# zhen6618/EPRecon

Measured on AMD Instinct MI355X. Metric: fragments_per_sec, higher is better.
Workload: dtype f32

## Files before the change

### eprecon_amd/_lib.py

```python
import ctypes
import os

import numpy as np
import torch

_HERE = os.path.dirname(os.path.abspath(__file__))
LIB_PATH = os.environ.get("EPRECON_LIB_PATH") or os.path.join(_HERE, "libeprecon_hip.so")

_c = ctypes
_vp, _i, _i64, _f, _sz = _c.c_void_p, _c.c_int, _c.c_int64, _c.c_float, _c.c_size_t

SIGNATURES = {
    "eprecon_abi_version": (_i, []),
    "eprecon_build_arch": (_c.c_char_p, []),
    "eprecon_back_project_workspace_bytes": (_sz, [_i64, _i, _i, _i, _i, _i, _i]),
    "eprecon_back_project_async": (_i, [_vp, _i64, _vp, _i, _f, _vp, _i, _vp, _i, _i, _i, _i, _i, _i,
                                        _vp, _vp, _vp, _vp, _vp, _vp, _vp, _vp, _sz, _vp]),
    "eprecon_back_project_call_async": (_i, [_vp, _vp]),
    "eprecon_back_project_call": (_i, [_vp, _i, _vp, _vp]),
    "eprecon_back_project_prepare_levels_async": (_i, [_vp, _i, _vp]),
    "eprecon_back_project_workspace_maps_offset": (_sz, [_i64, _i]),
    "eprecon_bp_levels": (_i, []),
    "eprecon_init_glue": (_i, []),
    "eprecon_profile_gather_kernel": (_c.c_char_p, []),
    "eprecon_hash_capacity": (_c.c_uint32, [_i64]),
    "eprecon_hash_table_bytes": (_sz, [_c.c_uint32]),
    "eprecon_hash_build_async": (_i, [_vp, _i64, _i, _vp, _c.c_uint32, _vp]),
    "eprecon_hash_build_dn_async": (_i, [_vp, _i64, _vp, _i, _vp, _c.c_uint32, _vp]),
    "eprecon_hash_query_async": (_i, [_vp, _c.c_uint32, _vp, _i64, _i, _vp, _vp]),
    "eprecon_hash_status": (_i, [_vp, _vp]),
    "eprecon_unique_workspace_bytes": (_sz, [_i64]),
    "eprecon_unique_coords_async": (_i, [_vp, _i64, _i, _vp, _c.c_uint32, _vp, _vp, _vp, _vp, _sz, _vp]),
    "eprecon_unique_coords_dn_async": (_i, [_vp, _i64, _vp, _i, _vp, _c.c_uint32, _vp, _vp, _vp, _vp, _sz, _vp]),
    "eprecon_unique_hierarchy_dn_async": (_i, [_vp, _i64, _vp, _i, _vp, _vp, _vp, _vp, _vp, _vp, _sz, _vp]),
    "eprecon_point_quantize_dn_async": (_i, [_vp, _i64, _vp, _f, _vp, _vp, _vp]),
    "eprecon_spvcnn_points_dn_async": (_i, [_vp, _i64, _vp, _i, _i, _vp, _i, _f, _vp, _f, _vp, _vp, _vp, _vp, _vp, _vp]),
    "eprecon_gru_stage_capacity": (_i64, [_vp, _i64, _i]),
    "eprecon_gru_stage_workspace_bytes": (_sz, [_i64]),
    "eprecon_gru_stage_begin_async": (_i, [_vp, _vp]),
    "eprecon_gru_stage_commit_async": (_i, [_vp, _vp, _vp, _vp]),
    "eprecon_kernel_map_async": (_i, [_vp, _c.c_uint32, _vp, _i64, _i, _i, _vp, _vp]),
    "eprecon_kernel_map_self_async": (_i, [_vp, _c.c_uint32, _vp, _i64, _i, _vp, _vp]),
    "eprecon_components_workspace_bytes": (_sz, [_i64]),
    "eprecon_components_async": (_i, [_vp, _i64, _vp, _i, _vp, _vp, _vp, _sz, _vp]),
    "eprecon_transpose_map_async": (_i, [_vp, _i64, _vp, _i, _vp, _vp]),
    "eprecon_sparse_conv_async": (_i, [_vp, _i64, _i, _vp, _i, _i64, _vp, _i, _i, _vp, _vp, _i, _i, _i, _vp]),
    "eprecon_conv_bn_partial_bytes": (_sz, [_i64, _i]),
    "eprecon_sparse_conv_fused_async": (_i, [_vp, _i64, _i, _vp, _i, _i64, _vp, _i, _i, _vp, _vp, _i, _vp, _i, _i, _i,
                                             _vp, _vp]),
    "eprecon_conv_desc_async": (_i, [_vp, _vp]),
    "eprecon_exclusive_scan_scratch_ints": (_sz, [_i64]),
    "eprecon_exclusive_scan_async": (_i, [_vp, _i64, _vp, _vp, _vp, _vp]),
    "eprecon_conv_desc_partial_rows": (_i64, [_vp]),
    "eprecon_conv_dense3d_kind": (_i, [_vp]),
    "eprecon_bn_acc_words": (_sz, [_i]),
    "eprecon_conv_desc_takes_bn_acc": (_i, [_vp]),
    "eprecon_batchnorm_acc_affine_async": (_i, [_vp, _i, _i, _i, _f, _vp, _vp, _vp]),
    "eprecon_affine_rows_acc_async": (_i, [_vp, _i64, _i, _i, _vp, _i, _i, _f, _i, _vp, _i, _vp]),
    "eprecon_affine_rows_res_async": (_i, [_vp, _i64, _i, _i, _vp, _vp, _vp, _i, _i, _vp, _i, _vp]),
    "eprecon_batchnorm_finalize_affine_async": (_i, [_vp, _i64, _i64, _i, _vp, _vp, _f, _vp, _vp, _vp]),
    "eprecon_affine_rows_async": (_i, [_vp, _i64, _i, _i, _vp, _vp, _i, _vp, _i, _vp]),
    "eprecon_affine_pool2_rows_async": (_i, [_vp, _i, _i, _i, _i, _i, _vp, _vp, _i, _vp, _i, _vp]),
    "eprecon_affine_up2_rows_async": (_i, [_vp, _i, _i, _i, _i, _i, _vp, _vp, _i, _vp, _i, _vp]),
    "eprecon_pixel_map_async": (_i, [_i, _i, _i, _i, _vp, _vp]),
    "eprecon_batchnorm_apply_workspace_bytes": (_sz, [_i]),
    "eprecon_batchnorm_apply_partials_async": (_i, [_vp, _i64, _i, _i, _vp, _i64, _i64, _vp, _vp, _f, _vp, _i, _i, _vp, _i,
                                                    _vp, _vp, _vp, _sz, _vp]),
    "eprecon_batchnorm_apply_partials_res_async": (_i, [_vp, _i64, _i, _i, _vp, _i64, _i64, _vp, _vp, _f, _vp, _i, _vp, _vp, _i,
                                                        _vp, _i, _vp, _sz, _vp]),
    "eprecon_batchnorm_workspace_bytes": (_sz, [_i64, _i]),
    "eprecon_batchnorm_train_async": (_i, [_vp, _i64, _i, _i, _vp, _vp, _f, _vp, _i, _i, _vp, _i, _vp, _vp,
                                           _vp, _sz, _vp]),
    "eprecon_rowwise_layernorm_async": (_i, [_vp, _i64, _i, _i, _vp, _i, _vp, _vp, _f, _i, _i, _vp, _i, _vp]),
    "eprecon_init_select_workspace_bytes": (_sz, [_i, _i]),
    "eprecon_init_select_async": (_i, [_vp, _vp, _i64, _f, _i, _i, _i, _vp, _vp, _vp, _sz, _vp]),
    "eprecon_init_select_dense_async": (_i, [_vp, _vp, _i64, _vp, _i, _i, _i, _i, _f, _i, _i, _vp, _vp, _vp, _sz, _vp]),
    "eprecon_upsample_async": (_i, [_vp, _i, _vp, _i64, _i, _i, _vp, _vp, _vp]),
    "eprecon_aligned_coords_async": (_i, [_vp, _i64, _vp, _i, _f, _vp, _vp, _vp]),
    "eprecon_point_quantize_async": (_i, [_vp, _i64, _f, _vp, _vp, _vp]),
    "eprecon_segment_workspace_bytes": (_sz, [_i64, _i64]),
    "eprecon_segment_lists_async": (_i, [_vp, _i64, _i64, _vp, _vp, _vp, _sz, _vp]),
    "eprecon_segment_mean_async": (_i, [_vp, _i, _vp, _vp, _i64, _i, _vp, _i, _vp]),
    "eprecon_sphash_async": (_i, [_vp, _i64, _vp, _vp]),
    "eprecon_sphash_order_workspace_bytes": (_sz, [_i64]),
    "eprecon_sphash_order_async": (_i, [_vp, _i64, _vp, _vp, _vp, _sz, _vp]),
    "eprecon_remap_index_async": (_i, [_vp, _i64, _vp, _vp, _i64, _vp, _vp]),
    "eprecon_trilinear_map_async": (_i, [_vp, _c.c_uint32, _vp, _i64, _i, _vp, _vp, _vp]),
    "eprecon_devoxelize_async": (_i, [_vp, _i, _vp, _vp, _i64, _i, _vp, _i, _i, _vp]),
    "eprecon_sparse_conv_wgrad_workspace_bytes": (_sz, [_i, _i64, _i, _i]),
    "eprecon_sparse_conv_wgrad_async": (_i, [_vp, _i, _vp, _i, _vp, _i, _i64, _i, _i, _vp, _vp, _sz, _vp]),
    "eprecon_invert_map_async": (_i, [_vp, _i, _i64, _i64, _vp, _vp]),
    "eprecon_devoxelize_backward_async": (_i, [_vp, _i, _vp, _vp, _i64, _i, _i64, _vp, _i, _vp]),
    "eprecon_gather_rows_scaled_async": (_i, [_vp, _i, _vp, _vp, _i64, _i, _vp, _i, _vp]),
    "eprecon_back_project_backward_async": (_i, [_vp, _i64, _vp, _i, _f, _vp, _vp, _i, _i, _i, _i, _i, _vp, _i, _vp, _vp, _vp]),
    "eprecon_back_project_backward_workspace_bytes": (_sz, [_i, _i, _i, _i, _i]),
    "eprecon_back_project_backward_det_async": (_i, [_vp, _i64, _vp, _i, _f, _vp, _vp, _i, _i, _i, _i, _i, _vp, _i, _vp, _vp, _vp, _sz,
                                                     _vp]),
    "eprecon_devoxelize_backward_csr_async": (_i, [_vp, _i, _vp, _vp, _vp, _i64, _i, _vp, _i, _vp]),
    "eprecon_devoxelize_gate_async": (_i, [_vp, _i, _vp, _vp, _i64, _i, _vp, _i, _i, _vp, _i, _vp, _i, _vp, _i, _vp]),
    "eprecon_devoxelize_gate_tail_async": (_i, [_vp, _i, _vp, _vp, _i64, _i, _vp, _i, _i, _vp, _i, _vp, _i, _vp, _i, _vp, _i, _vp, _i,
                                                _i, _vp]),
    "eprecon_fbv_union_workspace_bytes": (_sz, [_i]),
    "eprecon_fbv_union_async": (_i, [_vp, _vp, _i64, _i, _vp, _vp, _i64, _i, _i, _i, _i, _i, _vp, _vp, _vp, _vp, _vp,
                                     _vp, _vp, _sz, _vp]),
    "eprecon_map_set_fragment": (_i, [_vp, _i]),
    "eprecon_map_stamps_async": (_i, [_vp, _vp, _vp, _i, _c.c_int32, _vp]),
    "eprecon_map_select_boundary_async": (_i, [_vp, _vp, _i, _i, _i, _vp, _vp]),
    "eprecon_map_pack_boundary_async": (_i, [_vp, _vp, _i64, _vp]),
    "eprecon_map_merge_boundary": (_i, [_vp, _vp, _i64, _vp, _i, _vp, _vp]),
    "eprecon_map_create": (_i, [_i, _c.POINTER(_vp)]),
    "eprecon_map_destroy": (_i, [_vp]),
    "eprecon_map_reset": (_i, [_vp]),
    "eprecon_map_size": (_i64, [_vp]),
    "eprecon_map_channels": (_i, [_vp]),
    "eprecon_map_export_async": (_i, [_vp, _vp, _vp, _vp]),
    "eprecon_map_import_async": (_i, [_vp, _vp, _vp, _i64, _vp]),
    "eprecon_map_crop_union": (_i, [_vp, _vp, _vp, _i64, _i, _i, _i, _i, _vp, _vp, _vp, _vp, _vp, _vp]),
    "eprecon_map_gather_async": (_i, [_vp, _vp, _i64, _i, _i, _f, _vp, _i, _vp]),
    "eprecon_map_update_async": (_i, [_vp, _vp, _i64, _vp, _i, _vp]),
    "eprecon_map_target_fuse": (_i, [_vp, _vp, _vp, _i, _vp, _vp, _i64, _vp, _vp]),
    "eprecon_gather_rows_async": (_i, [_vp, _i, _vp, _i64, _i, _f, _vp, _i, _vp]),
    "eprecon_tsdf_integrate_async": (_i, [_vp, _vp, _vp, _vp, _f, _vp, _i, _i, _i, _vp, _vp, _f, _f, _i, _vp, _vp]),
    "eprecon_gt_crop_async": (_i, [_vp, _vp]),
    "eprecon_label_volumes_workspace_bytes": (_sz, [_i64, _i64]),
    "eprecon_label_volumes": (_i, [_vp, _vp, _vp, _vp, _i64, _vp, _c.c_double, _vp, _vp, _vp, _vp, _vp, _sz, _vp]),
    "eprecon_label_fill_workspace_bytes": (_sz, [_i, _i, _i]),
    "eprecon_label_fill_async": (_i, [_vp, _vp, _vp, _vp, _sz, _vp]),
    "eprecon_marching_cubes_table": (_i, [_vp]),
    "eprecon_marching_cubes_workspace_bytes": (_sz, [_i, _i, _i]),
    "eprecon_marching_cubes_count": (_i, [_vp, _i, _i, _i, _f, _vp, _vp, _sz, _vp]),
    "eprecon_marching_cubes_emit_async": (_i, [_vp, _i, _i, _i, _f, _vp, _vp, _vp, _vp, _vp, _vp, _vp, _vp, _vp]),
    "eprecon_marching_cubes_count_masked": (_i, [_vp, _vp, _i, _i, _i, _f, _vp, _vp, _sz, _vp]),
    "eprecon_marching_cubes_emit_masked_async": (_i, [_vp, _vp, _i, _i, _i, _f, _vp, _vp, _vp, _vp, _vp, _vp, _vp, _vp, _vp]),
# ... 404 lines not shown
```

### eprecon_amd/csrc/conv_common.hpp

```cpp
#pragma once
#include "common.hpp"

namespace epconv {

struct ConvParams {
    const float *x;
    const int32_t *nbr;
    const float *w;
    const float *bias;
    float *out;
    int n_out, K, Cin, Cout, ld_x, ld_out;
    int64_t x_bytes;
    int relu;
    int accumulate;
    const float *res;
    int ld_res;
    float *bn_partial;
    int bn_ld;
    const float *in_scale, *in_shift;
    int in_relu;
    const float *res_scale, *res_shift;
    int res_relu;
    int ln;
    const float *ln_gamma, *ln_beta;
    float ln_eps;
    int ln_post_relu;
    int img_h, img_w, img_maps;
    int flex_partial;
    const int32_t *vox_rank;
    int gx, gy, gz;
    const float *wq;
    const float *wq16;
    int debug;
    int splitk_pipe;
    void *ws;
    size_t ws_bytes;
    long long *bn_acc;
    int bn_acc_ld, bn_acc_c0;
    const float *bn_gamma, *bn_beta;
    const long long *in_acc;
    int in_acc_ld, in_acc_c0;
    float in_eps;
};

constexpr int kBnCopies = 8, kBnWords = 7;
#ifndef EP_BN_ABL
#define EP_BN_ABL 0
#endif

__device__ __forceinline__ void bn_limbs(double x, long long &l0, long long &l1, long long &l2)
{
    const double v = x * 1099511627776.0;
    const double hi = floor(v * (1.0 / 1099511627776.0));
    l0 = (long long)(v - hi * 1099511627776.0);
    const long long h = (long long)hi;
    l1 = h & ((1ll << 40) - 1);
    l2 = h >> 40;
}

__device__ __forceinline__ void bn_acc_add(long long *acc, int ld, int c, int copy, float n, float mean, float m2)
{
    if (n <= 0.0f || (EP_BN_ABL & 1)) return;
    unsigned long long *a = reinterpret_cast<unsigned long long *>(acc) + ((size_t)copy * ld + c) * kBnWords;
    const double dn = (double)n, dm = (double)mean;
    long long l0, l1, l2;
    bn_limbs(dn * dm, l0, l1, l2);
    atomicAdd(a + 0, (unsigned long long)l0);
    if (EP_BN_ABL & 4) return;
    atomicAdd(a + 1, (unsigned long long)l1); atomicAdd(a + 2, (unsigned long long)l2);
    bn_limbs((double)m2 + dn * dm * dm, l0, l1, l2);
    atomicAdd(a + 3, (unsigned long long)l0); atomicAdd(a + 4, (unsigned long long)l1); atomicAdd(a + 5, (unsigned long long)l2);
    atomicAdd(a + 6, (unsigned long long)(long long)n);
}

__device__ __forceinline__ void bn_acc_affine(const long long *acc, int ld, int c, float eps, float &scale, float &shift)
{
    if (EP_BN_ABL & 2) { scale = 1.0f; shift = 0.0f; return; }
    long long w[kBnWords] = {0, 0, 0, 0, 0, 0, 0};
#pragma unroll 1
    for (int k = 0; k < kBnCopies; ++k) {
        const long long *a = acc + ((size_t)k * ld + c) * kBnWords;
#pragma unroll
        for (int j = 0; j < kBnWords; ++j) w[j] += a[j];
    }
    const double two40 = 1099511627776.0;
    const double s1 = ((double)w[2] * two40 + (double)w[1]) + (double)w[0] * (1.0 / two40);
    const double s2 = ((double)w[5] * two40 + (double)w[4]) + (double)w[3] * (1.0 / two40);
    const double n = (double)w[6];
    const float *gb = reinterpret_cast<const float *>(acc + (size_t)kBnCopies * ld * kBnWords);
    const double mean = n > 0.0 ? s1 / n : 0.0;
    double var = n > 0.0 ? s2 / n - mean * mean : 0.0;
    if (var < 0.0) var = 0.0;
    const float sc = gb[c] / sqrtf((float)var + eps);
    scale = sc;
    shift = gb[ld + c] - (float)mean * sc;
}

template <int THREADS, bool ACC = true>
__device__ __forceinline__ void stage_in_affine(const ConvParams &p, float *sAff, int cpad, int tid)
{
    if (!p.in_scale) return;
    for (int c = tid; c < cpad; c += THREADS) {
        float sc = 0.0f, sh = 0.0f;
        if (c < p.Cin) {
            if (ACC && p.in_acc) bn_acc_affine(p.in_acc, p.in_acc_ld, p.in_acc_c0 + c, p.in_eps, sc, sh);
            else { sc = p.in_scale[c]; sh = p.in_shift[c]; }
        }
        sAff[c] = sc;
        sAff[cpad + c] = sh;
    }
}

__device__ __forceinline__ void bn_acc_publish(const ConvParams &p, int col, int copy, bool first, float n, float mean, float m2)
{
    bn_acc_add(p.bn_acc, p.bn_acc_ld, p.bn_acc_c0 + col, copy & (kBnCopies - 1), n, mean, m2);
    if (first) {
        float *gb = reinterpret_cast<float *>(p.bn_acc + (size_t)kBnCopies * p.bn_acc_ld * kBnWords);
        gb[p.bn_acc_c0 + col] = p.bn_gamma ? p.bn_gamma[col] : 1.0f;
        gb[p.bn_acc_ld + p.bn_acc_c0 + col] = p.bn_beta ? p.bn_beta[col] : 0.0f;
    }
}

constexpr int kWaves = 4;
constexpr int kRowsPerWave = 32;
constexpr int kRowsPerBlock = kRowsPerWave * kWaves;
typedef float f32x4 __attribute__((ext_vector_type(4)));
typedef unsigned int u32x4 __attribute__((ext_vector_type(4)));
// ... 72 lines not shown
            }
#pragma unroll
            for (int m = 8; m > 0; m >>= 1) sq += __shfl_xor(sq, m);
            const float inv = 1.0f / sqrtf(sq * inv_c + p.ln_eps);
#pragma unroll
            for (int t = 0; t < CT; ++t) {
                const int col = 16 * t + l16;
                float y = fmaf(v[t][j] * inv, (p.ln_gamma && colok[t]) ? p.ln_gamma[col] : 1.0f, (p.ln_beta && colok[t]) ? p.ln_beta[col] : 0.0f);
                if (p.ln_post_relu) y = fmaxf(y, 0.0f);
                v[t][j] = y;
            }
        }
    }
#pragma unroll
    for (int t = 0; t < CT; ++t)
#pragma unroll
        for (int j = 0; j < 4; ++j)
            if (colok[t] && orow[j] >= 0) p.out[(size_t)orow[j] * p.ld_out + 16 * t + l16] = v[t][j];
    if (p.bn_partial || (ACC && p.bn_acc)) {
#pragma unroll
        for (int t = 0; t < CT; ++t) {
            float n = 0.0f, sum = 0.0f;
#pragma unroll
            for (int j = 0; j < 4; ++j)
                if (orow[j] >= 0) { n += 1.0f; sum += v[t][j]; }
            float mean = n > 0.0f ? sum / n : 0.0f, m2 = 0.0f;
#pragma unroll
            for (int j = 0; j < 4; ++j)
                if (orow[j] >= 0) { const float d = v[t][j] - mean; m2 = fmaf(d, d, m2); }
#pragma unroll
            for (int m = 16; m < 64; m <<= 1) {
                const float on = __shfl_xor(n, m), om = __shfl_xor(mean, m), oq = __shfl_xor(m2, m);
                const bool lower = (lane & m) == 0;
                float a_n = lower ? n : on, a_mean = lower ? mean : om, a_m2 = lower ? m2 : oq;
                chan_merge(a_n, a_mean, a_m2, lower ? on : n, lower ? om : mean, lower ? oq : m2);
                n = a_n; mean = a_mean; m2 = a_m2;
            }
            if (q == 0) {
                float *d = sStat + (wave * 3) * 16 * CT + 16 * t + l16;
                d[0] = n; d[16 * CT] = mean; d[2 * 16 * CT] = m2;
            }
        }
        __syncthreads();
        if (tid < 16 * CT && tid < p.Cout) {
            float a_n = 0.0f, a_mean = 0.0f, a_m2 = 0.0f;
#pragma unroll
            for (int w = 0; w < NW; ++w)
                chan_merge(a_n, a_mean, a_m2, sStat[(w * 3) * 16 * CT + tid], sStat[(w * 3 + 1) * 16 * CT + tid], sStat[(w * 3 + 2) * 16 * CT + tid]);
            if (p.bn_partial) bn_partial_store(p, partial_row, tid, a_n, a_mean, a_m2);
            if (ACC && p.bn_acc) bn_acc_publish(p, tid, partial_row, partial_row == 0, a_n, a_mean, a_m2);
        }
    }
}

inline bool gather_vec4(const ConvParams &p)
{
    return (p.ld_x % 4 == 0) && ((reinterpret_cast<uintptr_t>(p.x) & 15) == 0) && (p.Cin % 4 == 0 || p.ld_x >= ((p.Cin + 3) & ~3));
}

enum D3Kind { kD3None = 0, kD3Narrow = 1, kD3Tile16 = 2 };
__attribute__((visibility("hidden"))) int conv3d_shape_kind(const ConvParams &p);
int conv3d_kind(const ConvParams &p);
int d3_tiles_kind(const ConvParams &p, int kind, int *ty = nullptr, int *tz = nullptr);
int launch_conv3d_16(const ConvParams &p, hipStream_t st);
int launch_conv3d_single_column(const ConvParams &p, hipStream_t st);

bool conv2d_tile_ok(const ConvParams &p, int *nt_out, int *nch_out, int64_t *blocks);
int launch_image_tile(const ConvParams &p, hipStream_t st);

constexpr int kWideRows = 128;
size_t wide_workspace_bytes(const ConvParams &p);
bool wide_shape_ok(const ConvParams &p);
bool wide_ok(const ConvParams &p);
int launch_wide(const ConvParams &p, hipStream_t st);

constexpr int kSplitKRows = 32;
bool splitk_ok(const ConvParams &p);
int launch_splitk(ConvParams &p, hipStream_t st);

bool resident_narrow_ok(const ConvParams &p);
int launch_resident_narrow(const ConvParams &p, hipStream_t st);
bool resident_wide_ok(const ConvParams &p);
int launch_resident_wide(const ConvParams &p, hipStream_t st);
int launch_mfma(const ConvParams &p, hipStream_t st);

bool direct16_ok(const ConvParams &p);
constexpr int kDirectRows = 128;
int launch_direct16(const ConvParams &p, hipStream_t st);
int direct16_partial_block_rows(const ConvParams &p);
size_t direct16_workspace_bytes(const ConvParams &p);

constexpr int kT2MinRows = 40000;
constexpr int kDirectMaxCout = 64;
constexpr int64_t kK1DirectMinRows = 20000;
bool tile2d16_ok(const ConvParams &p);
int64_t tile2d16_partial_rows(const ConvParams &p);
int launch_tile2d16(const ConvParams &p, hipStream_t st);

constexpr int kT2ShortMaxRows = 20000;
bool tile2d_short_list(const ConvParams &p);
bool tile2d_short_ok(const ConvParams &p);
int64_t tile2d_short_partial_rows(const ConvParams &p);
int launch_tile2d_short(const ConvParams &p, hipStream_t st);


}
```

### eprecon_amd/csrc/norm.hip

```cpp
#include <stdlib.h>

#include "common.hpp"
#include "conv_common.hpp"

namespace {
using namespace ep;

constexpr int kBnPerThread = 8;

__device__ __forceinline__ void chan_merge(float &n_a, float &mean_a, float &m2_a, float n_b, float mean_b, float m2_b)
{
    if (n_b == 0.0f) return;
    if (n_a == 0.0f) {
        n_a = n_b; mean_a = mean_b; m2_a = m2_b;
        return;
    }
    const float n = n_a + n_b;
    const float d = mean_b - mean_a;
    mean_a = mean_a + d * (n_b / n);
    m2_a = m2_a + m2_b + d * d * (n_a * n_b / n);
    n_a = n;
}

__global__ __launch_bounds__(256) void bn_stats_kernel(const float *x, int n, int C, int ld, float *partial)
// ... 12 lines not shown
        const bool ok = active && r < n;
        v[k] = ok ? x[(size_t)r * ld + col] : 0.0f;
        cnt += ok ? 1.0f : 0.0f;
        sum += v[k];
    }
    const float mean = cnt > 0.0f ? sum / cnt : 0.0f;
    float m2 = 0.0f;
#pragma unroll
    for (int k = 0; k < kBnPerThread; ++k) {
        const int r = r0 + k * rpi + rsub;
        if (active && r < n) {
            const float d = v[k] - mean;
            m2 = fmaf(d, d, m2);
        }
    }
    sN[tid] = cnt; sMean[tid] = mean; sM2[tid] = m2;
    __syncthreads();
    for (int s = 1; s < rpi; s <<= 1) {
        if (active && (rsub % (2 * s)) == 0 && rsub + s < rpi) {
            float n = sN[tid], m = sMean[tid], q = sM2[tid];
            const int o = tid + s * C;
            chan_merge(n, m, q, sN[o], sMean[o], sM2[o]);
            sN[tid] = n; sMean[tid] = m; sM2[tid] = q;
        }
        __syncthreads();
    }
    if (tid < C) {
        const size_t plane = (size_t)C * gridDim.x;
        float *p = partial + (size_t)tid * gridDim.x + blockIdx.x;
        p[0] = sN[tid]; p[plane] = sMean[tid]; p[2 * plane] = sM2[tid];
    }
}

template <int NU>
__device__ __forceinline__ void bn_merge_rows(const float *partial, int nblk, int64_t ld, int C, int c, int tid, float &a_n,
                                              float &a_mean, float &a_m2)
{
    const float *pn = partial + (size_t)c * ld, *pm = pn + (size_t)C * ld, *pq = pm + (size_t)C * ld;
    for (int b = tid; b < nblk; b += NU * 256) {
        float vn[NU], vm[NU], vq[NU];
#pragma unroll
        for (int u = 0; u < NU; ++u) {
            const int bb = b + u * 256;
            const bool ok = bb < nblk;
            vn[u] = ok ? pn[bb] : 0.0f;
            vm[u] = ok ? pm[bb] : 0.0f;
            vq[u] = ok ? pq[bb] : 0.0f;
        }
#pragma unroll
        for (int u = 0; u < NU; ++u) chan_merge(a_n, a_mean, a_m2, vn[u], vm[u], vq[u]);
    }
}

inline int bn_finalize_nu(int64_t nblk)
{
    const int64_t need = (nblk + 255) / 256;
    return need <= 1 ? 1 : need <= 2 ? 2 : need <= 4 ? 4 : need <= 8 ? 8 : 16;
}

template <int NU>
__global__ __launch_bounds__(256) void bn_finalize_kernel(const float *partial, int nblk, int64_t ld, int C, float *mean_out,
                                                          float *var_out)
{
    __shared__ float sN[256], sMean[256], sM2[256];
    const int c = blockIdx.x, tid = threadIdx.x;
    float a_n = 0.0f, a_mean = 0.0f, a_m2 = 0.0f;
    bn_merge_rows<NU>(partial, nblk, ld, C, c, tid, a_n, a_mean, a_m2);
    sN[tid] = a_n; sMean[tid] = a_mean; sM2[tid] = a_m2;
    __syncthreads();
    for (int s = 128; s > 0; s >>= 1) {
        if (tid < s) {
            float n = sN[tid], m = sMean[tid], q = sM2[tid];
            chan_merge(n, m, q, sN[tid + s], sMean[tid + s], sM2[tid + s]);
            sN[tid] = n; sMean[tid] = m; sM2[tid] = q;
        }
        __syncthreads();
    }
    if (tid == 0) {
        mean_out[c] = sMean[0];
        var_out[c] = sN[0] > 0.0f ? sM2[0] / sN[0] : 0.0f;
    }
}

template <int NU>
__global__ __launch_bounds__(256) void bn_finalize_affine_kernel(const float *partial, int nblk, int64_t ld, int C,
                                                                 const float *gamma, const float *beta, float eps,
                                                                 float *scale_out, float *shift_out)
{
    __shared__ float sN[4], sMean[4], sM2[4];
    const int c = blockIdx.x, tid = threadIdx.x;
    const float g_c = gamma ? gamma[c] : 1.0f, b_c = beta ? beta[c] : 0.0f;
    float a_n = 0.0f, a_mean = 0.0f, a_m2 = 0.0f;
    bn_merge_rows<NU>(partial, nblk, ld, C, c, tid, a_n, a_mean, a_m2);
    const int lane = tid & 63;
#pragma unroll
    for (int m = 1; m < 64; m <<= 1) {
        const float on = __shfl_xor(a_n, m), om = __shfl_xor(a_mean, m), oq = __shfl_xor(a_m2, m);
        float ln = (lane & m) ? on : a_n, lm = (lane & m) ? om : a_mean, lq = (lane & m) ? oq : a_m2;
        chan_merge(ln, lm, lq, (lane & m) ? a_n : on, (lane & m) ? a_mean : om, (lane & m) ? a_m2 : oq);
        a_n = ln; a_mean = lm; a_m2 = lq;
    }
    if (lane == 0) { sN[tid >> 6] = a_n; sMean[tid >> 6] = a_mean; sM2[tid >> 6] = a_m2; }
    __syncthreads();
    if (tid == 0) {
        float n = sN[0], mean = sMean[0], m2 = sM2[0];
        for (int w = 1; w < 4; ++w) chan_merge(n, mean, m2, sN[w], sMean[w], sM2[w]);
        const float var = n > 0.0f ? m2 / n : 0.0f;
        const float sc = g_c / sqrtf(var + eps);
        scale_out[c] = sc;
        shift_out[c] = b_c - mean * sc;
    }
}

__global__ __launch_bounds__(256) void bn_apply_kernel(const float *x, int n, int C, int ld_x,
                                                       const float *mean, const float *var,
                                                       const float *gamma, const float *beta, float eps,
                                                       const float *res, int ld_res, const float *res_scale,
                                                       const float *res_shift, int relu, float *out, int ld_out)
{
    const size_t e = (size_t)blockIdx.x * 256 + threadIdx.x;
    if (e >= (size_t)n * C) return;
    const int r = (int)(e / C), c = (int)(e - (size_t)r * C);
    const float inv = 1.0f / sqrtf(var[c] + eps);
    float v = (x[(size_t)r * ld_x + c] - mean[c]) * inv;
    v = v * (gamma ? gamma[c] : 1.0f) + (beta ? beta[c] : 0.0f);
    if (res) {
        float rv = res[(size_t)r * ld_res + c];
        if (res_scale) rv = fmaf(rv, res_scale[c], res_shift[c]);
        v += rv;
    }
    if (relu) v = fmaxf(v, 0.0f);
    out[(size_t)r * ld_out + c] = v;
}

__global__ __launch_bounds__(256) void rowwise_ln_kernel(const float *x, int n, int C, int ld_x,
                                                         const float *res, int ld_res,
                                                         const float *gamma, const float *beta, float eps,
                                                         int pre_relu, int post_relu, float *out,
                                                         int ld_out)
{
    const int g = threadIdx.x & 7;
    const int r = blockIdx.x * 32 + (threadIdx.x >> 3);
    const bool live = r < n;
    const float *xr = x + (size_t)(live ? r : 0) * ld_x;
    const float *rr = res ? res + (size_t)(live ? r : 0) * ld_res : nullptr;
    auto value = [&](int c) -> float {
        float v = xr[c];
        if (pre_relu) v = fmaxf(v, 0.0f);
        if (rr) v += rr[c];
        return v;
    };
    float s = 0.0f;
    if (live)
        for (int c = g; c < C; c += 8) s += value(c);
    s += __shfl_xor(s, 1);
    s += __shfl_xor(s, 2);
    s += __shfl_xor(s, 4);
    const float mean = s / (float)C;
    float q = 0.0f;
    if (live)
        for (int c = g; c < C; c += 8) {
            const float d = value(c) - mean;
            q = fmaf(d, d, q);
        }
    q += __shfl_xor(q, 1);
    q += __shfl_xor(q, 2);
    q += __shfl_xor(q, 4);
    const float inv = 1.0f / sqrtf(q / (float)C + eps);
    if (live)
        for (int c = g; c < C; c += 8) {
            float v = (value(c) - mean) * inv * (gamma ? gamma[c] : 1.0f) + (beta ? beta[c] : 0.0f);
// ... 217 lines not shown
    return EPRECON_OK;
}

}

extern "C" {

static inline int bn_rows_per_block(int channels) { return kBnPerThread * (256 / channels); }

size_t eprecon_batchnorm_workspace_bytes(int64_t n, int channels)
{
    if (channels <= 0 || channels > 256) return 0;
    const size_t nblk = (size_t)ceil_div(n > 0 ? n : 1, bn_rows_per_block(channels));
    return align_up(nblk * 3 * channels * sizeof(float), 256) + 2 * align_up((size_t)channels * sizeof(float), 256);
}

int eprecon_batchnorm_train_async(const float *x, int64_t n, int channels, int ld_x, const float *gamma,
                                  const float *beta, float eps, const float *residual, int ld_res,
                                  int relu, float *out, int ld_out, float *mean_out, float *var_out,
                                  void *workspace, size_t workspace_bytes, void *stream)
{
    if (!x || !out || n < 0 || channels <= 0 || channels > 256 || ld_x < channels || ld_out < channels ||
        !workspace)
        return EPRECON_ERR_ARG;
    if (workspace_bytes < eprecon_batchnorm_workspace_bytes(n, channels)) return EPRECON_ERR_WORKSPACE;
    if (n == 0) return EPRECON_OK;
    hipStream_t st = (hipStream_t)stream;
    const int nblk = (int)ceil_div(n, bn_rows_per_block(channels));
    char *ws = reinterpret_cast<char *>(workspace);
    float *partial = reinterpret_cast<float *>(ws);
    ws += align_up((size_t)nblk * 3 * channels * sizeof(float), 256);
    float *mean = mean_out ? mean_out : reinterpret_cast<float *>(ws);
    ws += align_up((size_t)channels * sizeof(float), 256);
    float *var = var_out ? var_out : reinterpret_cast<float *>(ws);
    hipLaunchKernelGGL(bn_stats_kernel, dim3(nblk), dim3(256), 0, st, x, (int)n, channels, ld_x, partial);
    EP_LAUNCH_CHECK();
    return bn_finalize_apply(x, n, channels, ld_x, partial, nblk, nblk, gamma, beta, eps, residual, ld_res, relu, out,
                             ld_out, mean, var, st);
}

size_t eprecon_batchnorm_apply_workspace_bytes(int channels)
{
    return 2 * align_up((size_t)(channels > 0 ? channels : 1) * sizeof(float), 256);
}

int eprecon_batchnorm_apply_partials_async(const float *x, int64_t n, int channels, int ld_x,
                                           const float *partial, int64_t nblk, int64_t ld, const float *gamma,
                                           const float *beta, float eps, const float *residual,
                                           int ld_res, int relu, float *out, int ld_out, float *mean_out,
                                           float *var_out, void *workspace, size_t workspace_bytes,
                                           void *stream)
{
    if (!x || !out || !partial || n < 0 || nblk <= 0 || nblk > 0x7fffffff || ld < nblk || channels <= 0 || ld_x < channels ||
        ld_out < channels || !workspace)
        return EPRECON_ERR_ARG;
    if (workspace_bytes < eprecon_batchnorm_apply_workspace_bytes(channels)) return EPRECON_ERR_WORKSPACE;
    if (n == 0) return EPRECON_OK;
    char *ws = reinterpret_cast<char *>(workspace);
    float *mean = mean_out ? mean_out : reinterpret_cast<float *>(ws);
    ws += align_up((size_t)channels * sizeof(float), 256);
    float *var = var_out ? var_out : reinterpret_cast<float *>(ws);
    return bn_finalize_apply(x, n, channels, ld_x, partial, (int)nblk, ld, gamma, beta, eps, residual, ld_res, relu,
                             out, ld_out, mean, var, (hipStream_t)stream);
}

int eprecon_batchnorm_apply_partials_res_async(const float *x, int64_t n, int channels, int ld_x, const float *partial,
                                               int64_t nblk, int64_t ld, const float *gamma, const float *beta, float eps,
                                               const float *residual, int ld_res, const float *res_scale,
                                               const float *res_shift, int relu, float *out, int ld_out, void *workspace,
                                               size_t workspace_bytes, void *stream)
{
    if (!x || !out || !partial || !residual || !res_scale || !res_shift || n < 0 || nblk <= 0 || nblk > 0x7fffffff || ld < nblk ||
        channels <= 0 || ld_x < channels || ld_out < channels || ld_res < channels || !workspace)
        return EPRECON_ERR_ARG;
    if (workspace_bytes < eprecon_batchnorm_apply_workspace_bytes(channels)) return EPRECON_ERR_WORKSPACE;
    if (n == 0) return EPRECON_OK;
    char *ws = reinterpret_cast<char *>(workspace);
    float *mean = reinterpret_cast<float *>(ws);
    float *var = reinterpret_cast<float *>(ws + align_up((size_t)channels * sizeof(float), 256));
    return bn_finalize_apply(x, n, channels, ld_x, partial, (int)nblk, ld, gamma, beta, eps, residual, ld_res, relu, out, ld_out,
                             mean, var, (hipStream_t)stream, res_scale, res_shift);
}

int eprecon_batchnorm_finalize_affine_async(const float *partial, int64_t nblk, int64_t ld, int channels, const float *gamma,
                                            const float *beta, float eps, float *scale_out, float *shift_out,
                                            void *stream)
{
    if (!partial || !scale_out || !shift_out || nblk <= 0 || nblk > 0x7fffffff || ld < nblk || channels <= 0) return EPRECON_ERR_ARG;
    hipStream_t st = (hipStream_t)stream;
    switch (bn_finalize_nu(nblk)) {
#define EP_FINALIZE(NU)                                                                                                            \
    case NU:                                                                                                                       \
        hipLaunchKernelGGL(bn_finalize_affine_kernel<NU>, dim3(channels), dim3(256), 0, st, partial, (int)nblk, ld, channels, gamma, \
                           beta, eps, scale_out, shift_out);                                                                         \
        break
        EP_FINALIZE(1); EP_FINALIZE(2); EP_FINALIZE(4); EP_FINALIZE(8); EP_FINALIZE(16);
#undef EP_FINALIZE
    }
    EP_LAUNCH_CHECK();
    return EPRECON_OK;
}

int eprecon_affine_rows_async(const float *x, int64_t n, int channels, int ld_x, const float *scale,
                              const float *shift, int relu, float *out, int ld_out, void *stream)
{
    if (!x || !out || !scale || !shift || n < 0 || channels <= 0 || ld_x < channels || ld_out < channels ||
        n * channels > 0x7fffffffll * 256)
        return EPRECON_ERR_ARG;
    if (n == 0) return EPRECON_OK;
    hipLaunchKernelGGL(affine_rows_kernel, dim3((unsigned)ceil_div(n * channels, (int64_t)256)), dim3(256), 0,
                       (hipStream_t)stream, x, (int)n, channels, ld_x, scale, shift, relu, out, ld_out);
    EP_LAUNCH_CHECK();
    return EPRECON_OK;
}

static bool rows_vec4(const float *x, int ld_x, const float *out, int ld_out, int channels)
{
    return channels % 4 == 0 && ld_x % 4 == 0 && ld_out % 4 == 0 && ((uintptr_t)x | (uintptr_t)out) % 16 == 0;
}

int eprecon_affine_pool2_rows_async(const float *x, int maps, int height, int width, int channels, int ld_x, const float *scale,
                                    const float *shift, int relu, float *out, int ld_out, void *stream)
{
    if (!x || !out || !scale || !shift || maps <= 0 || height < 2 || width < 2 || channels <= 0 || ld_x < channels ||
        ld_out < channels || (int64_t)maps * height * width * channels > 0x7fffffffll)
        return EPRECON_ERR_ARG;
    const bool v4 = rows_vec4(x, ld_x, out, ld_out, channels);
    const int64_t total = (int64_t)maps * (height / 2) * (width / 2) * (channels / (v4 ? 4 : 1));
    const dim3 grid((unsigned)ceil_div(total, (int64_t)256));
    if (v4)
        hipLaunchKernelGGL(affine_pool2_rows_kernel<4>, grid, dim3(256), 0, (hipStream_t)stream, x, maps, height, width, channels,
                           ld_x, scale, shift, relu, out, ld_out);
    else
        hipLaunchKernelGGL(affine_pool2_rows_kernel<1>, grid, dim3(256), 0, (hipStream_t)stream, x, maps, height, width, channels,
                           ld_x, scale, shift, relu, out, ld_out);
    EP_LAUNCH_CHECK();
    return EPRECON_OK;
}

int eprecon_affine_up2_rows_async(const float *x, int maps, int height, int width, int channels, int ld_x, const float *scale,
                                  const float *shift, int relu, float *out, int ld_out, void *stream)
{
    if (!x || !out || !scale || !shift || maps <= 0 || height <= 0 || width <= 0 || channels <= 0 || ld_x < channels ||
        ld_out < channels || (int64_t)maps * height * width * 4 * channels > 0x7fffffffll)
        return EPRECON_ERR_ARG;
    const bool v4 = rows_vec4(x, ld_x, out, ld_out, channels);
    const int64_t total = (int64_t)maps * 4 * height * width * (channels / (v4 ? 4 : 1));
    const dim3 grid((unsigned)ceil_div(total, (int64_t)256));
    if (v4)
        hipLaunchKernelGGL(affine_up2_rows_kernel<4>, grid, dim3(256), 0, (hipStream_t)stream, x, maps, height, width, channels,
                           ld_x, scale, shift, relu, out, ld_out);
    else
        hipLaunchKernelGGL(affine_up2_rows_kernel<1>, grid, dim3(256), 0, (hipStream_t)stream, x, maps, height, width, channels,
                           ld_x, scale, shift, relu, out, ld_out);
    EP_LAUNCH_CHECK();
    return EPRECON_OK;
}

int eprecon_batchnorm_acc_affine_async(const long long *acc, int acc_ld, int acc_c0, int channels, float eps, float *scale_out,
                                       float *shift_out, void *stream)
{
    if (!acc || !scale_out || !shift_out || channels <= 0 || acc_c0 < 0 || acc_c0 + channels > acc_ld) return EPRECON_ERR_ARG;
    hipLaunchKernelGGL(bn_acc_affine_kernel, dim3((unsigned)ceil_div(channels, 256)), dim3(256), 0, (hipStream_t)stream, acc, acc_ld,
                       acc_c0, channels, eps, scale_out, shift_out);
    EP_LAUNCH_CHECK();
    return EPRECON_OK;
}

int eprecon_affine_rows_acc_async(const float *x, int64_t n, int channels, int ld_x, const long long *acc, int acc_ld, int acc_c0,
                                  float eps, int relu, float *out, int ld_out, void *stream)
{
    if (!x || !out || !acc || n < 0 || channels <= 0 || channels > kAccRowsMaxC || ld_x < channels || ld_out < channels ||
        acc_c0 < 0 || acc_c0 + channels > acc_ld || n * channels > 0x7fffffffll * 256)
        return EPRECON_ERR_ARG;
    if (n == 0) return EPRECON_OK;
    hipLaunchKernelGGL(affine_rows_acc_kernel, dim3((unsigned)ceil_div(n * channels, (int64_t)4096)), dim3(256), 0,
                       (hipStream_t)stream, x, (int)n, channels, ld_x, acc, acc_ld, acc_c0, eps, relu, out, ld_out);
    EP_LAUNCH_CHECK();
    return EPRECON_OK;
}

int eprecon_affine_rows_res_async(const float *x, int64_t n, int channels, int ld_x, const float *scale,
                                  const float *shift, const float *residual, int ld_res, int relu, float *out,
// ... 28 lines not shown
```

### eprecon_amd/csrc/sparse_conv.hip

```cpp
#include <stdio.h>
#include <stdlib.h>

#include "common.hpp"
#include "conv_common.hpp"

namespace {
using namespace ep;
using namespace epconv;

struct ConvProf {
    bool armed = false, recorded = false;
    int K = 0, cin = 0, cout = 0;
    int64_t min_rows = 0, rows = 0;
    const char *kernel = "";
    hipEvent_t start = nullptr, stop = nullptr;
    unsigned long long *pairs_dev = nullptr;
} g_conv_prof;

__global__ void count_map_pairs_kernel(const int32_t *nbr, size_t total, unsigned long long *out)
{
    unsigned long long c = 0;
    for (size_t e = (size_t)blockIdx.x * blockDim.x + threadIdx.x; e < total; e += (size_t)gridDim.x * blockDim.x) c += nbr[e] >= 0;
    for (int m = 32; m > 0; m >>= 1) c += __shfl_xor(c, m);
    if ((threadIdx.x & 63) == 0 && c) atomicAdd(out, c);
// ... 122 lines not shown
    g.rows = p.n_out;
    g.kernel = g_last_conv_kernel;
    if (g.pairs_dev) {
        EP_HIP_CHECK(hipMemsetAsync(g.pairs_dev, 0, 2 * sizeof(unsigned long long), st));
        if (family == kFamDense3dNarrow || family == kFamDense3dTile16)
            hipLaunchKernelGGL(count_grid_pairs_kernel, dim3(256), dim3(256), 0, st, p.vox_rank, p.gx, p.gy, p.gz, g.pairs_dev);
        else if (p.nbr) {
            hipLaunchKernelGGL(count_map_pairs_kernel, dim3(256), dim3(256), 0, st, p.nbr, (size_t)p.K * p.n_out, g.pairs_dev);
            if (family == kFamDirect16)
                hipLaunchKernelGGL(count_map_groups_kernel, dim3(256), dim3(256), 0, st, p.nbr, p.n_out, p.K, g.pairs_dev + 1);
        } else
            EP_HIP_CHECK(hipMemcpyAsync(g.pairs_dev, &g.rows, sizeof(unsigned long long), hipMemcpyHostToDevice, st));
        EP_LAUNCH_CHECK();
    }
    return rc;
}

}

__global__ void profile_mark_kernel() {}
extern "C" int eprecon_profile_mark_async(int id, void *stream)
{
    hipStream_t st = static_cast<hipStream_t>(stream);
    hipLaunchKernelGGL(profile_mark_kernel, dim3((unsigned)id + 1), dim3(64), 0, st);
    EP_LAUNCH_CHECK();
    return EPRECON_OK;
}

extern "C" int eprecon_profile_conv_arm(int kvol, int cin, int cout, int64_t min_rows)
{
    ConvProf &g = g_conv_prof;
    if (!g.start) {
        EP_HIP_CHECK(hipEventCreate(&g.start));
        EP_HIP_CHECK(hipEventCreate(&g.stop));
        EP_HIP_CHECK(hipMalloc(&g.pairs_dev, 2 * sizeof(unsigned long long)));
    }
    g.K = kvol; g.cin = cin; g.cout = cout; g.min_rows = min_rows;
    g.armed = true;
    g.recorded = false;
    return EPRECON_OK;
}

extern "C" float eprecon_profile_conv_ms(int64_t *rows_out, const char **kernel_out)
{
    ConvProf &g = g_conv_prof;
    if (!g.recorded || hipEventSynchronize(g.stop) != hipSuccess) return -1.0f;
    float ms = -1.0f;
    if (hipEventElapsedTime(&ms, g.start, g.stop) != hipSuccess) return -1.0f;
    if (rows_out) *rows_out = g.rows;
    if (kernel_out) *kernel_out = g.kernel;
    return ms;
}

extern "C" const char *eprecon_profile_last_conv_kernel(void) { return g_last_conv_kernel; }

extern "C" int64_t eprecon_profile_conv_pairs(void)
{
    ConvProf &g = g_conv_prof;
    if (!g.recorded || !g.pairs_dev || hipEventSynchronize(g.stop) != hipSuccess) return -1;
    unsigned long long v = 0;
    if (hipMemcpy(&v, g.pairs_dev, sizeof(v), hipMemcpyDeviceToHost) != hipSuccess) return -1;
    return (int64_t)v;
}

extern "C" int64_t eprecon_profile_conv_executed_pairs(void)
{
    ConvProf &g = g_conv_prof;
    if (!g.recorded || !g.pairs_dev || hipEventSynchronize(g.stop) != hipSuccess) return -1;
    unsigned long long v = 0;
    if (hipMemcpy(&v, g.pairs_dev + 1, sizeof(v), hipMemcpyDeviceToHost) != hipSuccess) return -1;
    return (int64_t)v;
}

extern "C" size_t eprecon_conv_bn_partial_bytes(int64_t n_out, int cout)
{
    return (size_t)ep::ceil_div(n_out > 0 ? n_out : 1, (int64_t)128) * 3 * (size_t)(cout > 0 ? cout : 1) * sizeof(float);
}

static int64_t conv_x_bytes(const ConvParams &p, int64_t n_in)
{
    return n_in > 0 ? ((n_in - 1) * (int64_t)p.ld_x + ((p.Cin + 3) & ~3)) * 4 : 0;
}

static int conv_check_and_run(ConvParams &p, int64_t n_in, int64_t n_out, void *stream)
{
    if (!p.x || !p.w || !p.out || n_in < 0 || n_out < 0 || p.K <= 0 || p.K > 64 || p.Cin <= 0 || p.Cout <= 0 ||
        p.ld_x < p.Cin || p.ld_out < p.Cout || (p.res && p.ld_res < p.Cout))
        return EPRECON_ERR_ARG;
    if (!p.nbr && !p.vox_rank && p.K != 1) return EPRECON_ERR_ARG;
    if (!p.nbr && n_in != n_out) return EPRECON_ERR_ARG;
    if ((p.in_scale == nullptr) != (p.in_shift == nullptr) || (p.res_scale == nullptr) != (p.res_shift == nullptr))
        return EPRECON_ERR_ARG;
    if (p.Cout > 4096 || n_out > 0x7fffffff) return EPRECON_ERR_UNSUPPORTED;
    if (n_out == 0) return EPRECON_OK;
    p.n_out = (int)n_out;
    p.x_bytes = conv_x_bytes(p, n_in);
    return conv_dispatch(p, (hipStream_t)stream);
}

static void params_from_desc(ConvParams &p, const eprecon_conv_desc *d)
{
    p.x = d->x; p.nbr = d->nbr; p.w = d->weight; p.bias = d->bias; p.out = d->out;
    p.K = d->kvol; p.Cin = d->cin; p.Cout = d->cout; p.ld_x = d->ld_x; p.ld_out = d->ld_out;
    p.relu = d->relu; p.accumulate = d->accumulate;
    p.res = d->residual; p.ld_res = d->ld_res; p.bn_partial = d->bn_partial; p.bn_ld = d->bn_ld;
    p.in_scale = d->in_scale; p.in_shift = d->in_shift; p.in_relu = d->in_relu;
    p.res_scale = d->res_scale; p.res_shift = d->res_shift; p.res_relu = d->res_relu;
    p.ln = d->ln; p.ln_gamma = d->ln_gamma; p.ln_beta = d->ln_beta; p.ln_eps = d->ln_eps;
    p.ln_post_relu = d->ln_post_relu;
    p.img_h = d->img_h; p.img_w = d->img_w; p.img_maps = d->img_maps;
    p.vox_rank = d->vox_rank; p.gx = d->grid_x; p.gy = d->grid_y; p.gz = d->grid_z; p.wq = d->packed_weight;
    p.wq16 = d->packed_weight16;
    p.ws = d->workspace; p.ws_bytes = d->workspace_bytes;
    p.flex_partial = 1;
    p.bn_acc = d->bn_acc; p.bn_acc_ld = d->bn_acc_ld; p.bn_acc_c0 = d->bn_acc_c0; p.bn_gamma = d->bn_gamma; p.bn_beta = d->bn_beta;
    p.in_acc = d->in_acc; p.in_acc_ld = d->in_acc_ld; p.in_acc_c0 = d->in_acc_c0; p.in_eps = d->in_eps;
}

static bool query_params(ConvParams &p, const eprecon_conv_desc *d)
{
    if (!d) return false;
    params_from_desc(p, d);
    const bool rows = d->n_out > 0 && d->n_out <= 0x7fffffff;
    p.n_out = rows ? (int)d->n_out : 0;
    p.x_bytes = conv_x_bytes(p, d->n_in);
    return rows;
}

extern "C" int eprecon_batchnorm_acc_affine_async(const long long *acc, int acc_ld, int acc_c0, int channels, float eps,
                                                  float *scale_out, float *shift_out, void *stream);

static bool bn_acc_family(const ConvParams &p) { return conv3d_kind(p) == kD3None; }

extern "C" size_t eprecon_bn_acc_words(int ld)
{
    return ld > 0 ? (size_t)epconv::kBnCopies * ld * epconv::kBnWords + (size_t)(2 * ld + 1) / 2 : 0;
}

extern "C" int eprecon_conv_desc_takes_bn_acc(const eprecon_conv_desc *d)
{
    ConvParams p = {};
    return query_params(p, d) && !p.ln && !p.accumulate && bn_acc_family(p) ? 1 : 0;
}

extern "C" int eprecon_conv_dense3d_kind(const eprecon_conv_desc *d)
{
    ConvParams p = {};
    return query_params(p, d) ? conv3d_shape_kind(p) : kD3None;
}

extern "C" int64_t eprecon_conv_desc_partial_rows(const eprecon_conv_desc *d);

extern "C" int eprecon_conv_desc_async(const eprecon_conv_desc *d, void *stream)
{
    if (!d) return EPRECON_ERR_ARG;
    ConvParams p = {};
    query_params(p, d);
    if (p.bn_partial) {
        const int64_t rows = eprecon_conv_desc_partial_rows(d);
        if (p.bn_ld == 0) p.bn_ld = (int)(rows > 0 ? rows : 1);
        if (p.bn_ld < rows) return EPRECON_ERR_ARG;
    }
    if (p.bn_acc && (p.bn_acc_ld <= 0 || p.bn_acc_c0 < 0 || p.bn_acc_c0 + p.Cout > p.bn_acc_ld || p.ln || p.accumulate || !bn_acc_family(p)))
        return EPRECON_ERR_ARG;
    if (p.in_acc) {
        if (p.in_scale || p.in_shift || p.in_acc_ld <= 0 || p.in_acc_c0 < 0 || p.in_acc_c0 + p.Cin > p.in_acc_ld) return EPRECON_ERR_ARG;
        if (bn_acc_family(p)) {
            p.in_scale = p.in_shift = reinterpret_cast<const float *>(p.in_acc);
        } else {
            if (!d->in_affine_scratch) return EPRECON_ERR_ARG;
            const int rc = eprecon_batchnorm_acc_affine_async(p.in_acc, p.in_acc_ld, p.in_acc_c0, p.Cin, p.in_eps, d->in_affine_scratch,
                                                              d->in_affine_scratch + p.Cin, stream);
            if (rc != EPRECON_OK) return rc;
            p.in_scale = d->in_affine_scratch;
            p.in_shift = d->in_affine_scratch + p.Cin;
            p.in_acc = nullptr;
        }
    }
    return conv_check_and_run(p, d->n_in, d->n_out, stream);
}

extern "C" size_t eprecon_conv_desc_workspace_bytes(const eprecon_conv_desc *d)
{
    ConvParams p = {};
    if (!query_params(p, d)) return 0;
    const size_t wide = wide_shape_ok(p) ? wide_workspace_bytes(p) : 0;
    const size_t direct = select_conv(p).family == kFamDirect16 ? direct16_workspace_bytes(p) : 0;
    return wide > direct ? wide : direct;
}

extern "C" int64_t eprecon_conv_desc_partial_rows(const eprecon_conv_desc *d)
{
    ConvParams p = {};
    return query_params(p, d) ? select_conv(p).partial_rows : 0;
}

extern "C" int eprecon_sparse_conv_fused_async(const float *x, int64_t n_in, int ld_x, const int32_t *nbr,
                                               int kvol, int64_t n_out, const float *weight, int cin,
                                               int cout, const float *bias, const float *residual,
                                               int ld_res, float *out, int ld_out, int relu,
                                               int accumulate, float *bn_partial, void *stream)
{
    ConvParams p = {};
    p.x = x; p.nbr = nbr; p.w = weight; p.bias = bias; p.out = out;
    p.K = kvol; p.Cin = cin; p.Cout = cout; p.ld_x = ld_x; p.ld_out = ld_out;
    p.relu = relu; p.accumulate = accumulate;
    p.res = residual; p.ld_res = ld_res; p.bn_partial = bn_partial;
    p.bn_ld = (int)ep::ceil_div(n_out > 0 ? n_out : 1, (int64_t)kRowsPerBlock);
    return conv_check_and_run(p, n_in, n_out, stream);
}

extern "C" int eprecon_sparse_conv_async(const float *x, int64_t n_in, int ld_x, const int32_t *nbr,
                                         int kvol, int64_t n_out, const float *weight, int cin,
                                         int cout, const float *bias, float *out, int ld_out,
                                         int relu, int accumulate, void *stream)
{
    return eprecon_sparse_conv_fused_async(x, n_in, ld_x, nbr, kvol, n_out, weight, cin, cout, bias, nullptr, 0,
                                           out, ld_out, relu, accumulate, nullptr, stream);
}
```

### eprecon_amd/csrc/sparse_conv_direct.hip

```cpp
#include "sparse_conv_direct_select.hpp"

namespace epconv {
int launch_direct16_ct1(const ConvParams &p, hipStream_t st);
int launch_direct16_ct2(const ConvParams &p, hipStream_t st);
int launch_direct16_ct3(const ConvParams &p, hipStream_t st);
int launch_direct16_ct4(const ConvParams &p, hipStream_t st);

bool direct16_ok(const ConvParams &p)
{
    if (switch_off("EPRECON_CONV_DIRECT")) return false;
    const bool pointwise = p.K == 1 && !p.nbr;
    if (!pointwise && ((p.K != 27 && p.K != 9) || !p.nbr)) return false;
    if (!p.wq16 || (reinterpret_cast<uintptr_t>(p.wq16) & 15) != 0) return false;
    if (p.Cout > 64 || p.accumulate) return false;
    if (p.ld_x % 4 != 0 || (reinterpret_cast<uintptr_t>(p.x) & 15) != 0 || (p.Cin % 4 != 0 && p.ld_x < ((p.Cin + 3) & ~3))) return false;
    if (p.x_bytes <= 0 || p.x_bytes >= 0x7fffffffll || (int64_t)p.ld_x * 4 >= (1 << 24) || p.x_bytes / ((int64_t)p.ld_x * 4) >= (1 << 24))
        return false;
    return true;
}

int direct16_partial_block_rows(const ConvParams &p) { return persist_shape_ok(p) ? kJobRows : kDirectRows; }
size_t direct16_workspace_bytes(const ConvParams &p) { return persist_shape_ok(p) ? kPersistCtrBytes : 0; }

int launch_direct16(const ConvParams &p, hipStream_t st)
{
    switch ((p.Cout + 15) / 16) {
        case 1: return launch_direct16_ct1(p, st);
        case 2: return launch_direct16_ct2(p, st);
        case 3: return launch_direct16_ct3(p, st);
        default: return launch_direct16_ct4(p, st);
    }
}

}
```

### eprecon_amd/csrc/sparse_conv_direct_ct1.hip

```cpp
#include "sparse_conv_direct_launch.hpp"

namespace epconv {
int launch_direct16_ct1(const ConvParams &p, hipStream_t st) { return launch_ct<1>(p, st); }
}
```

### eprecon_amd/csrc/sparse_conv_direct_ct2.hip

```cpp
#include "sparse_conv_direct_launch.hpp"

namespace epconv {
int launch_direct16_ct2(const ConvParams &p, hipStream_t st) { return launch_ct<2>(p, st); }
}
```

### eprecon_amd/csrc/sparse_conv_direct_ct3.hip

```cpp
#include "sparse_conv_direct_launch.hpp"

namespace epconv {
int launch_direct16_ct3(const ConvParams &p, hipStream_t st) { return launch_ct<3>(p, st); }
}
```

### eprecon_amd/csrc/sparse_conv_direct_ct4.hip

```cpp
#include "sparse_conv_direct_launch.hpp"

namespace epconv {
int launch_direct16_ct4(const ConvParams &p, hipStream_t st) { return launch_ct<4>(p, st); }
}
```

### eprecon_amd/csrc/sparse_conv_direct_kernels.hpp

```cpp
#pragma once
#include "sparse_conv_direct_device.hpp"

namespace epconv {
namespace {

template <int CT, int KCH, bool TAIL = false, int G = stage_chunks(KCH), bool BF = false, int MODE = 0>
__global__ __launch_bounds__(256) void spconv_direct16_kernel(ConvParams p)
{
    extern __shared__ __attribute__((aligned(16))) char smem[];
    constexpr int RT = kRT, ROWS = kDirectRows;
    constexpr int CTM = TAIL ? CT - 1 : CT;
    constexpr int CTA = CTM > 0 ? CTM : 1;
    constexpr int PARTS = KCH / G;
    constexpr int cpad = 16 * KCH;
    int *sNbr = reinterpret_cast<int *>(smem);
    float *sStat = reinterpret_cast<float *>(sNbr + p.K * ROWS);
    float *sAff = sStat + kWaves * 3 * 16 * CT;
    int *sFlag = reinterpret_cast<int *>(sAff + 2 * cpad);
    const int tid = threadIdx.x;
    const int lane = tid & 63, wave = tid >> 6;
    const int l16 = lane & 15, q = lane >> 4;
    const int row0 = (int)blockIdx.x * ROWS;

    stage_in_affine<256>(p, sAff, cpad, tid);
    const unsigned live = stage_map(p, row0, sNbr, sFlag, tid);

    static_assert(!(BF && TAIL), "the bf16x3 form runs on padded column tiles");
    static_assert(MODE < 3 || (G == KCH && !BF), "modes 3 / 4: one stage per offset, exact-fp32 form");

    constexpr int NS = (CTM == 1 && !BF) ? 2 : 1;
    f32x4 acc[NS][RT][CTA];
    f32x4 acct[RT][2];
#pragma unroll
    for (int rt = 0; rt < RT; ++rt) {
#pragma unroll
        for (int ns = 0; ns < NS; ++ns)
#pragma unroll
            for (int t = 0; t < CTA; ++t) acc[ns][rt][t] = f32x4{0.0f, 0.0f, 0.0f, 0.0f};
        acct[rt][0] = acct[rt][1] = f32x4{0.0f, 0.0f, 0.0f, 0.0f};
    }

    const __amdgpu_buffer_rsrc_t xrsrc = __builtin_amdgcn_make_buffer_rsrc(const_cast<float *>(p.x), 0, (int)p.x_bytes, 0x00020000);
    const unsigned row_bytes = (unsigned)p.ld_x * 4u, oob = (unsigned)p.x_bytes;
    const int U = __builtin_popcount(live) * PARTS;
    constexpr unsigned kChunkBytes = (unsigned)CT * 1024u;
    const __amdgpu_buffer_rsrc_t wrsrc =
        __builtin_amdgcn_make_buffer_rsrc(const_cast<float *>(p.wq16), 0, (int)((unsigned)p.K * KCH * kChunkBytes), 0x00020000);
    const unsigned wlane = (unsigned)lane * 16u;
    const __amdgpu_buffer_rsrc_t wtrsrc = __builtin_amdgcn_make_buffer_rsrc(
        const_cast<float *>(p.wq16) + (size_t)p.K * KCH * CT * 256, 0, (int)((unsigned)p.K * KCH * 512u), 0x00020000);
    const unsigned tlane = (unsigned)(4 * q + (lane & 3)) * 16u;
    const int *myNbr = sNbr + wave * 16 * RT + l16;
    const int last_c = p.Cin - 16 * (KCH - 1);
    const bool tail8 = last_c <= 8;
    const unsigned cq = 16u * (unsigned)q;
    const unsigned cq_last = tail8 ? 8u * (unsigned)q : cq;
    const bool last_ok = (tail8 ? 2 : 4) * q < last_c;

    struct Stage {
        float4 a[G][RT];
        float4 b[G][CTA];
        float4 bt[G][TAIL ? 2 : 1];
    };
    auto fetch = [&](const LiveCursor &c, Stage &g) {
        const int k = c.k, part = c.part;
        const unsigned xs = 64u * (unsigned)(part * G);
        const unsigned ws = (EP_DIRECT_ABL & 8) ? 0u : (unsigned)(k * KCH + part * G) * kChunkBytes;
        const bool has_last = part == PARTS - 1;
#pragma unroll
        for (int rt = 0; rt < RT; ++rt) {
            int j = myNbr[k * ROWS + 16 * rt];
            if (EP_DIRECT_ABL & 2) j = j >= 0 ? l16 : j;
            const unsigned rowsel = j >= 0 ? __umul24((unsigned)j, row_bytes) : oob;
            const unsigned v0 = rowsel + cq;
#pragma unroll
            for (int i = 0; i < G; ++i) {
                unsigned off = v0 + 64u * i;
                if (i == G - 1 && has_last) off = last_ok ? rowsel + cq_last + 64u * i : oob;
                if (EP_DIRECT_ABL & 4) {
                    g.a[i][rt] = make_float4(__uint_as_float(off), 1.0f, 2.0f, 3.0f);
                    continue;
                }
                const u32x4 v = __builtin_amdgcn_raw_buffer_load_b128(xrsrc, off, xs, 0);
                g.a[i][rt] = make_float4(__uint_as_float(v.x), __uint_as_float(v.y), __uint_as_float(v.z), __uint_as_float(v.w));
            }
        }
#pragma unroll
        for (int i = 0; i < G; ++i) {
#pragma unroll
            for (int t = 0; t < CTM; ++t) {
                if (EP_DIRECT_ABL & 32) {
                    g.b[i][t] = make_float4(__uint_as_float(ws), 1.0f, 2.0f, 3.0f);
// ... 345 lines not shown
```

### eprecon_amd/csrc/sparse_conv_direct_launch.hpp

```cpp
#pragma once
#include "sparse_conv_direct_kernels.hpp"
#include "sparse_conv_direct_persist.hpp"

namespace epconv {
namespace {

template <int CT, int KCH>
int launch_form(const DirectForm &f, const ConvParams &p, dim3 grid, size_t lds, hipStream_t st)
{
    constexpr int G0 = stage_chunks(KCH), GA = alt_stage_chunks(KCH);
    if (f.persist) {
        if constexpr (KCH * (CT * 1024 - 512) <= 4864) {
            if (f.tail) return launch_persist<CT, KCH, true>(p, st);
            if constexpr (KCH * CT * 1024 <= 4864) return launch_persist<CT, KCH, false>(p, st);
        }
        return EPRECON_ERR_UNSUPPORTED;
    }
    void (*kern)(ConvParams) = nullptr;
    auto with_tail = [&](auto tail) {
        constexpr bool TAIL = decltype(tail)::value;
        if (f.bf) {
            if constexpr (!TAIL)
                kern = f.mode == 2   ? spconv_direct16_kernel<CT, KCH, false, G0, true, 2>
                       : f.mode == 1 ? spconv_direct16_kernel<CT, KCH, false, G0, true, 1>
                                     : spconv_direct16_kernel<CT, KCH, false, G0, true>;
        } else if (f.g != G0) {
            if constexpr (GA != 0) kern = spconv_direct16_kernel<CT, KCH, TAIL, GA>;
        } else if (f.mode >= 3) {
            if constexpr (G0 == KCH)
                kern = f.mode == 4 ? spconv_direct16_kernel<CT, KCH, TAIL, G0, false, 4> : spconv_direct16_kernel<CT, KCH, TAIL, G0, false, 3>;
        } else {
            kern = f.mode == 2   ? spconv_direct16_kernel<CT, KCH, TAIL, G0, false, 2>
                   : f.mode == 1 ? spconv_direct16_kernel<CT, KCH, TAIL, G0, false, 1>
                                 : spconv_direct16_kernel<CT, KCH, TAIL, G0>;
        }
    };
    if (f.tail) with_tail(std::true_type{});
    else with_tail(std::false_type{});
    if (!kern) return EPRECON_ERR_UNSUPPORTED;
    hipLaunchKernelGGL(kern, grid, dim3(256), lds, st, p);
    EP_LAUNCH_CHECK();
    return EPRECON_OK;
}

template <int CT, int KCH>
void stage_occupancy(bool tail, size_t lds, int &occ_p, int &occ_a)
{
    constexpr int G0 = stage_chunks(KCH), GA = alt_stage_chunks(KCH);
    static int occ[2][2] = {{0, 0}, {0, 0}};
    int *o = occ[tail ? 1 : 0];
    if (!o[0]) {
        const void *kp = tail ? reinterpret_cast<const void *>(spconv_direct16_kernel<CT, KCH, true, G0>)
                              : reinterpret_cast<const void *>(spconv_direct16_kernel<CT, KCH, false, G0>);
        const void *ka = tail ? reinterpret_cast<const void *>(spconv_direct16_kernel<CT, KCH, true, GA>)
                              : reinterpret_cast<const void *>(spconv_direct16_kernel<CT, KCH, false, GA>);
        int a = 0, b = 0;
        if (hipOccupancyMaxActiveBlocksPerMultiprocessor(&a, kp, 256, lds) != hipSuccess || a <= 0) a = 1;
        if (hipOccupancyMaxActiveBlocksPerMultiprocessor(&b, ka, 256, lds) != hipSuccess || b <= 0) b = a;
        o[1] = b;
        o[0] = a;
    }
    occ_p = o[0];
    occ_a = o[1];
}

template <int CT, int KCH>
int launch_k(const ConvParams &p, hipStream_t st)
{
    const size_t lds = direct_lds_bytes(p.K, CT, KCH);
    const DirectSwitches sw = direct_switches();
    int occ_p = 1, occ_a = 1;
    if constexpr (alt_stage_chunks(KCH) != 0) stage_occupancy<CT, KCH>(direct_tail(p, sw), lds, occ_p, occ_a);
    const DirectForm f = select_direct_form(p, sw, device_cus(), occ_p, occ_a);
    return launch_form<CT, KCH>(f, p, dim3((unsigned)ceil_div(p.n_out, kDirectRows)), lds, st);
}

template <int CT>
int launch_ct(const ConvParams &p, hipStream_t st)
{
    const int kch = (p.Cin + 15) / 16;
    if (kch <= 6) return pick<1, 2, 3, 4, 5, 6>(kch, [&](auto k) { return launch_k<CT, decltype(k)::value>(p, st); });
    hipLaunchKernelGGL((spconv_direct16_generic_kernel<CT>), dim3((unsigned)ceil_div(p.n_out, kDirectRows)), dim3(256),
                       direct_lds_bytes(p.K, CT, kch), st, p, kch);
    EP_LAUNCH_CHECK();
    return EPRECON_OK;
}

}
}
```

### eprecon_amd/csrc/sparse_conv_slab.hip

```cpp
#include "common.hpp"
#include "conv_common.hpp"
#include "conv_gather.hpp"

namespace {
using namespace ep;
using namespace epconv;

template <int NT, bool VEC4>
__global__ __launch_bounds__(256) void spconv_mfma_kernel(ConvParams p)
{
    extern __shared__ __attribute__((aligned(16))) char smem[];
    constexpr int TN = 32 * NT;
    float *sW = reinterpret_cast<float *>(smem);
    int *sNbr = reinterpret_cast<int *>(sW + 2 * kSlabC * TN);
    int *sActive = sNbr + p.K * kRowsPerBlock;
    const int cinA = (p.Cin + 3) & ~3;
    float *sAff = reinterpret_cast<float *>(sActive + ((p.K + 3) & ~3));

    const int tid = threadIdx.x;
    const int lane = tid & 63, wave = tid >> 6;
    const int r32 = lane & 31, half = lane >> 5;
    const int row0 = blockIdx.x * kRowsPerBlock;
    const int col0 = blockIdx.y * TN;

    for (int k = tid; k < p.K; k += 256) sActive[k] = 0;
    stage_in_affine<256>(p, sAff, cinA, tid);
    __syncthreads();
    for (int e = tid; e < p.K * kRowsPerBlock; e += 256) {
        const int k = e / kRowsPerBlock, r = e - k * kRowsPerBlock;
        const int row = row0 + r;
        int j = -1;
        if (row < p.n_out) j = p.nbr ? p.nbr[(size_t)k * p.n_out + row] : row;
        sNbr[e] = j;
        if (j >= 0) sActive[k] = 1;
    }
    __syncthreads();

    f32x16 acc[NT];
#pragma unroll
    for (int t = 0; t < NT; ++t)
#pragma unroll
        for (int r = 0; r < 16; ++r) acc[t][r] = 0.0f;

    const int nslab = (p.Cin + kSlabC - 1) / kSlabC;
    int buf = 0;
    bool have_prev = false;
    for (int k = 0; k < p.K; ++k) {
        if (!sActive[k]) continue;
        const int j = sNbr[k * kRowsPerBlock + wave * kRowsPerWave + r32];
        const float *xrow = p.x + (size_t)(j >= 0 ? j : 0) * p.ld_x;
        const float *wk = p.w + (size_t)k * p.Cin * p.Cout + col0;
        for (int sl = 0; sl < nslab; ++sl) {
            const int c0 = sl * kSlabC;
            float *dstW = sW + buf * kSlabC * TN;
            stage_weights<TN>(dstW, wk, c0, p.Cin, p.Cout, p.Cout - col0, kSlabC, tid);
            float a[4][4];
#pragma unroll
            for (int ch = 0; ch < 4; ++ch) {
                const int c = c0 + ch * 8 + 4 * half;
                if (VEC4) {
                    float4 v = make_float4(0.f, 0.f, 0.f, 0.f);
                    if (j >= 0 && c < p.Cin) v = *reinterpret_cast<const float4 *>(xrow + c);
                    if (p.Cin & 3) {
                        if (c + 1 >= p.Cin) v.y = 0.0f;
                        if (c + 2 >= p.Cin) v.z = 0.0f;
                        if (c + 3 >= p.Cin) v.w = 0.0f;
                    }
                    a[ch][0] = v.x; a[ch][1] = v.y; a[ch][2] = v.z; a[ch][3] = v.w;
                } else {
#pragma unroll
                    for (int s = 0; s < 4; ++s) a[ch][s] = (j >= 0 && c + s < p.Cin) ? xrow[c + s] : 0.0f;
                }
            }
            __syncthreads();
            (void)have_prev;
            const float *srcW = sW + buf * kSlabC * TN;
            const int nch = min(4, (p.Cin - c0 + 7) / 8);
            if (p.in_scale) {
#pragma unroll
                for (int ch = 0; ch < 4; ++ch) {
                    const int c = c0 + ch * 8 + 4 * half;
#pragma unroll
                    for (int s = 0; s < 4; ++s) {
                        const bool ok = j >= 0 && c + s < p.Cin;
                        float v = fmaf(a[ch][s], sAff[min(c + s, cinA - 1)], sAff[cinA + min(c + s, cinA - 1)]);
                        if (p.in_relu) v = fmaxf(v, 0.0f);
                        a[ch][s] = ok ? v : 0.0f;
                    }
                }
            }
            for (int ch = 0; ch < nch; ++ch) {
#pragma unroll
                for (int s = 0; s < 4; ++s) {
                    const float *brow = srcW + (ch * 8 + 4 * half + s) * TN + r32;
#pragma unroll
                    for (int t = 0; t < NT; ++t)
                        acc[t] = __builtin_amdgcn_mfma_f32_32x32x2f32(a[ch][s], brow[t * 32], acc[t], 0, 0, 0);
                }
            }
            buf ^= 1;
            have_prev = true;
        }
    }

    conv_epilogue<NT>(p, acc, LinearRows{row0 + wave * kRowsPerWave, p.n_out}, col0, r32, half, wave, sW, (int)blockIdx.x, (int)gridDim.y);
}

template <int NT>
int launch_conv(const ConvParams &p, bool vec4, hipStream_t st)
{
    const dim3 grid((unsigned)ceil_div(p.n_out, kRowsPerBlock), (unsigned)ceil_div(p.Cout, 32 * NT));
    const size_t lds = (size_t)2 * kSlabC * 32 * NT * sizeof(float) +
                       (size_t)p.K * kRowsPerBlock * sizeof(int) + (size_t)((p.K + 3) & ~3) * sizeof(int) +
                       (size_t)2 * ((p.Cin + 3) & ~3) * sizeof(float) + 16;
    if (vec4)
        hipLaunchKernelGGL((spconv_mfma_kernel<NT, true>), grid, dim3(256), lds, st, p);
    else
        hipLaunchKernelGGL((spconv_mfma_kernel<NT, false>), grid, dim3(256), lds, st, p);
    EP_LAUNCH_CHECK();
    return EPRECON_OK;
}

constexpr int kTileH = 8, kTileW = 16;
constexpr int kHaloH = kTileH + 2, kHaloW = kTileW + 2;

template <int NT, int NCH>
__global__ __launch_bounds__(256) void conv2d_tile_kernel(ConvParams p, int tiles_x, int tiles_y)
{
    constexpr int cin_pad = NCH * 8;
    constexpr int P = cin_pad + 4;
    constexpr int TN = 32 * NT;
    extern __shared__ __attribute__((aligned(16))) char smem[];
    float *sW = reinterpret_cast<float *>(smem);
    float *sX = sW + 9 * cin_pad * TN;
    const int tid = threadIdx.x;
    const int lane = tid & 63, wave = tid >> 6;
    const int r32 = lane & 31, half = lane >> 5;
    const int tx = blockIdx.x % tiles_x, ty = blockIdx.x / tiles_x, map = blockIdx.y;
    const int col0 = blockIdx.z * TN;
    const int x0 = tx * kTileW, y0 = ty * kTileH;
    const size_t map_row0 = (size_t)map * p.img_h * p.img_w;

    __shared__ __attribute__((aligned(16))) float sInAff[2 * cin_pad];
    if (p.in_acc) {
        stage_in_affine<256>(p, sInAff, cin_pad, tid);
        __syncthreads();
    }
    if (cin_pad == p.Cin) {
        stage_weights<TN>(sW, p.w + col0, 0, 9 * p.Cin, p.Cout, p.Cout - col0, 9 * cin_pad, tid);
    } else {
        for (int k = 0; k < 9; ++k)
            stage_weights<TN>(sW + k * cin_pad * TN, p.w + col0, k * p.Cin, (k + 1) * p.Cin, p.Cout, p.Cout - col0, cin_pad, tid);
    }
    constexpr int C4 = cin_pad / 4;
    constexpr int kHaloItems = kHaloH * kHaloW * C4;
    constexpr int kHaloIter = (kHaloItems + 255) / 256;
    float4 hv[kHaloIter];
#pragma unroll
    for (int it = 0; it < kHaloIter; ++it) {
        const int e = min(tid + it * 256, kHaloItems - 1);
        const int px = e / C4, c4 = e - px * C4;
        const int hy = px / kHaloW, hx = px - hy * kHaloW;
        const int y = min(max(y0 - 1 + hy, 0), p.img_h - 1), x = min(max(x0 - 1 + hx, 0), p.img_w - 1);
        hv[it] = *reinterpret_cast<const float4 *>(p.x + (map_row0 + (size_t)y * p.img_w + x) * p.ld_x + min(c4 * 4, p.Cin - 4));
    }
#pragma unroll
    for (int it = 0; it < kHaloIter; ++it) {
        const int e = tid + it * 256;
        if (e >= kHaloItems) break;
        const int px = e / C4, c4 = e - px * C4;
        const int hy = px / kHaloW, hx = px - hy * kHaloW;
        const int y = y0 - 1 + hy, x = x0 - 1 + hx;
        const int c = c4 * 4;
        float4 v = hv[it];
        if (p.in_scale) {
            float4 sc, sh;
            if (p.in_acc) {
                sc = *reinterpret_cast<const float4 *>(sInAff + min(c, cin_pad - 4));
                sh = *reinterpret_cast<const float4 *>(sInAff + cin_pad + min(c, cin_pad - 4));
            } else {
                sc = *reinterpret_cast<const float4 *>(p.in_scale + min(c, p.Cin - 4));
                sh = *reinterpret_cast<const float4 *>(p.in_shift + min(c, p.Cin - 4));
            }
            v.x = fmaf(v.x, sc.x, sh.x); v.y = fmaf(v.y, sc.y, sh.y);
            v.z = fmaf(v.z, sc.z, sh.z); v.w = fmaf(v.w, sc.w, sh.w);
            if (p.in_relu) {
                v.x = fmaxf(v.x, 0.f); v.y = fmaxf(v.y, 0.f); v.z = fmaxf(v.z, 0.f); v.w = fmaxf(v.w, 0.f);
            }
        }
        if (!(y >= 0 && y < p.img_h && x >= 0 && x < p.img_w && c < p.Cin)) v = make_float4(0.f, 0.f, 0.f, 0.f);
        *reinterpret_cast<float4 *>(sX + px * P + c) = v;
    }
    __syncthreads();

    f32x16 acc[NT];
#pragma unroll
    for (int t = 0; t < NT; ++t)
#pragma unroll
        for (int r = 0; r < 16; ++r) acc[t][r] = 0.0f;

    const int ry = 2 * wave + (r32 >> 4), rx = r32 & 15;
// ... 15 lines not shown
                for (int t = 0; t < NT; ++t) b[q][t] = wk[(ch * 8 + q) * TN + t * 32];
#pragma unroll
            for (int t = 0; t < NT; ++t) {
                acc[t] = __builtin_amdgcn_mfma_f32_32x32x2f32(av[ch].x, b[0][t], acc[t], 0, 0, 0);
                acc[t] = __builtin_amdgcn_mfma_f32_32x32x2f32(av[ch].y, b[1][t], acc[t], 0, 0, 0);
                acc[t] = __builtin_amdgcn_mfma_f32_32x32x2f32(av[ch].z, b[2][t], acc[t], 0, 0, 0);
                acc[t] = __builtin_amdgcn_mfma_f32_32x32x2f32(av[ch].w, b[3][t], acc[t], 0, 0, 0);
            }
        }
    }
    const int wy0 = y0 + 2 * wave;
    const ImageRows rm{(int)(map_row0 + (size_t)wy0 * p.img_w + x0), wy0, x0, p.img_h, p.img_w};
    const int partial_row = ((int)blockIdx.y * tiles_y + ty) * tiles_x + tx;
    conv_epilogue<NT>(p, acc, rm, col0, r32, half, wave, sW, partial_row, (int)gridDim.z);
}

size_t conv2d_tile_lds(int nt, int nch) { return ((size_t)9 * nch * 8 * 32 * nt + (size_t)kHaloH * kHaloW * (nch * 8 + 4)) * sizeof(float); }

template <int NCH>
int launch_conv2d_tile(const ConvParams &p, hipStream_t st)
{
    const int tiles_x = (p.img_w + kTileW - 1) / kTileW, tiles_y = (p.img_h + kTileH - 1) / kTileH;
    const dim3 grid((unsigned)(tiles_x * tiles_y), (unsigned)p.img_maps, (unsigned)ceil_div(p.Cout, 32));
    const size_t lds = max(conv2d_tile_lds(1, NCH), (size_t)3 * 256 * sizeof(float));
    if (lds > 64 * 1024) {
        static const hipError_t attr = hipFuncSetAttribute(reinterpret_cast<const void *>(&conv2d_tile_kernel<1, NCH>),
                                                           hipFuncAttributeMaxDynamicSharedMemorySize, 96 * 1024);
        if (attr != hipSuccess) return EPRECON_ERR_HIP_BASE - (int)attr;
    }
    hipLaunchKernelGGL((conv2d_tile_kernel<1, NCH>), grid, dim3(256), lds, st, p, tiles_x, tiles_y);
    EP_LAUNCH_CHECK();
    return EPRECON_OK;
}

bool column_split(const ConvParams &p)
{
    return (int)ceil_div(p.n_out, kRowsPerBlock) < 256 && (p.Cout + 31) / 32 > 1 && !p.ln;
}
int cin_pad8(const ConvParams &p) { return (p.Cin + 7) / 8 * 8; }
}

namespace epconv {
bool conv2d_tile_ok(const ConvParams &p, int *nt_out, int *nch_out, int64_t *blocks)
{
    if (p.K != 9 || p.img_h <= 0 || p.img_w <= 0 || p.img_maps <= 0 || p.ln || p.accumulate)
        return false;
    if ((int64_t)p.img_maps * p.img_h * p.img_w != p.n_out) return false;
    if (p.Cin % 4 != 0 || p.ld_x % 4 != 0 || (reinterpret_cast<uintptr_t>(p.x) & 15) != 0) return false;
    if (p.in_scale && ((reinterpret_cast<uintptr_t>(p.in_scale) & 15) != 0 || (reinterpret_cast<uintptr_t>(p.in_shift) & 15) != 0))
        return false;
    const int nch = (p.Cin + 7) / 8;
    if (nch > 5) return false;
    const int nt = 1;
    if (conv2d_tile_lds(nt, nch) > 96 * 1024) return false;
    const int tiles = ((p.img_h + kTileH - 1) / kTileH) * ((p.img_w + kTileW - 1) / kTileW);
    if ((int64_t)tiles * p.img_maps < 256) return false;
    *nt_out = nt; *nch_out = nch; *blocks = (int64_t)tiles * p.img_maps;
    return true;
}

int launch_resident_nt1(const ConvParams &p, bool vec4, int cin_pad, hipStream_t st);
int launch_resident_nt2(const ConvParams &p, bool vec4, int cin_pad, hipStream_t st);

bool resident_narrow_ok(const ConvParams &p) { return cin_pad8(p) <= 64 && (p.Cout <= 64 || column_split(p)); }

int launch_resident_narrow(const ConvParams &p, hipStream_t st)
{
    return ((p.Cout + 31) / 32 == 1 || column_split(p)) ? launch_resident_nt1(p, gather_vec4(p), cin_pad8(p), st)
                                                        : launch_resident_nt2(p, gather_vec4(p), cin_pad8(p), st);
}

bool resident_wide_ok(const ConvParams &p)
{
    return cin_pad8(p) > 64 && gather_vec4(p) && (p.K == 27 || p.K == 8) && !(p.ln && (p.Cout + 31) / 32 > 2);
}

int launch_resident_wide(const ConvParams &p, hipStream_t st)
{
    const int nblk = (int)ceil_div(p.n_out, kRowsPerBlock), nt_full = (p.Cout + 31) / 32;
    const bool two = nt_full >= 2 && (p.ln || (int64_t)nblk * ((nt_full + 1) / 2) >= 256);
    return two ? launch_resident_nt2(p, gather_vec4(p), cin_pad8(p), st) : launch_resident_nt1(p, gather_vec4(p), cin_pad8(p), st);
}

int launch_mfma(const ConvParams &p, hipStream_t st)
{
    const bool vec4 = gather_vec4(p);
    const int nt_full = (p.Cout + 31) / 32;
    if (nt_full == 1 || column_split(p)) return launch_conv<1>(p, vec4, st);
    if (nt_full == 2) return launch_conv<2>(p, vec4, st);
    if (nt_full == 3) return launch_conv<3>(p, vec4, st);
    return launch_conv<4>(p, vec4, st);
}

int launch_image_tile(const ConvParams &p, hipStream_t st)
{
    switch ((p.Cin + 7) / 8) {
        case 1: return launch_conv2d_tile<1>(p, st);
        case 2: return launch_conv2d_tile<2>(p, st);
        case 3: return launch_conv2d_tile<3>(p, st);
        case 4: return launch_conv2d_tile<4>(p, st);
        default: return launch_conv2d_tile<5>(p, st);
    }
}

}
```

### eprecon_amd/dense2d.py

```python
import ctypes
import os

import torch

from . import _lib
from . import sparse as SP


class PixelGrid:
    _cache = {}

    def __init__(self, maps, height, width, device):
        self.maps, self.height, self.width, self.device = maps, height, width, device
        self.n = maps * height * width
        self._nbr = {}

    @classmethod
    def get(cls, maps, height, width, device):
        key = (maps, height, width, str(device))
        g = cls._cache.get(key)
        if g is None:
            g = cls._cache[key] = cls(maps, height, width, device)
        return g

# ... 44 lines not shown

    def __init__(self, device, words=1 << 19):
        self.buf = torch.zeros(words, dtype=torch.int64, device=device)
        self.offset = 0
        self.high = words

    def begin(self):
        if self.high:
            self.buf[:self.high].zero_()
        self.offset = 0
        self.high = 0

    def take(self, words):
        words = (words + 1) & ~1
        if self.offset + words > self.buf.numel():
            raise _lib.EpreconError("BatchNorm accumulator arena exhausted (eprecon_amd.dense2d.BnArena)")
        t = self.buf[self.offset:self.offset + words]
        self.offset += words
        self.high = max(self.high, self.offset)
        return t


_ARENA = None


class bn_pass:

    def __init__(self, arena):
        self.arena = arena

    def __enter__(self):
        global _ARENA
        self.prev, _ARENA = _ARENA, self.arena
        if self.arena is not None:
            self.arena.begin()
        return self.arena

    def __exit__(self, *exc):
        global _ARENA
        _ARENA = self.prev
        return False


class AccSlice:
    __slots__ = ("block", "ld", "c0", "c")

    def __init__(self, block, ld, c0, c):
        self.block, self.ld, self.c0, self.c = block, ld, c0, c

    @classmethod
    def new(cls, channels):
        words = int(_lib.load().eprecon_bn_acc_words(channels))
        return cls(_ARENA.take(words), channels, 0, channels)

    def part(self, a, b):
        return AccSlice(self.block, self.ld, self.c0 + a, b - a)


class Act:
    __slots__ = ("rows", "scale", "shift", "relu", "acc", "eps")

    def __init__(self, rows, scale=None, shift=None, relu=False, acc=None, eps=1e-5):
        self.rows, self.scale, self.shift, self.relu, self.acc, self.eps = rows, scale, shift, relu, acc, eps

    def affine(self):
        if self.acc is not None and self.scale is None:
            a = torch.empty((2, self.acc.c), dtype=torch.float32, device=self.rows.device)
            _lib.check(_lib.load().eprecon_batchnorm_acc_affine_async(
                self.acc.block.data_ptr(), self.acc.ld, self.acc.c0, self.acc.c, float(self.eps), a[0].data_ptr(), a[1].data_ptr(),
                _lib.current_stream()), "eprecon_batchnorm_acc_affine_async")
            self.scale, self.shift = a[0], a[1]
        return self.scale, self.shift


def _dptr(t):
    return None if t is None else t.data_ptr()


def conv_bn_act(conv, bn, x, grid, out=None, aff=None, relu=True, pre_relu=False, residual=None):
    return conv_bn_launch(packed_weight(conv), conv.bias, bn.weight, bn.bias, bn.eps, conv.kernel_size[0], x, grid,
                          out=out, aff=aff, relu=relu, pre_relu=pre_relu, residual=residual)


def conv_bn_launch(w, bias, gamma, beta, eps, k, x, grid, out=None, aff=None, relu=True, pre_relu=False,
                   residual=None):
    lib = _lib.load()
    cout = w.shape[2]
    dev = x.rows.device
    acc_in = x.acc is not None and x.scale is None
    out, _, d, _keep = SP.conv_call(
        x.rows, w, grid.kernel_map(k), bias, out, relu=pre_relu, residual=None if residual is None else residual.rows,
        res_affine=None if residual is None else (*residual.affine(), residual.relu),
        in_affine=(x.scale, x.shift, x.relu) if x.scale is not None or x.relu else None,
        in_acc=(x.acc, x.eps, x.relu) if acc_in else None,
        image=(grid.height, grid.width, grid.maps) if k == 3 else None, launch=False, k1_min_rows=K1_DIRECT_2D_MIN_ROWS,
        image_limits=(DIRECT_2D_MIN_ROWS, SHORT_2D_MAX_ROWS, SHORT_2D_MAX_COUT) if k == 3 else None)
    if _ARENA is not None and (aff is None or isinstance(aff, AccSlice)) and lib.eprecon_conv_desc_takes_bn_acc(ctypes.byref(d)):
        acc = aff if aff is not None else AccSlice.new(cout)
        assert acc.c == cout
        d.bn_acc, d.bn_acc_ld, d.bn_acc_c0 = acc.block.data_ptr(), acc.ld, acc.c0
        d.bn_gamma, d.bn_beta = _dptr(gamma), _dptr(beta)
        _lib.check(lib.eprecon_conv_desc_async(ctypes.byref(d), _lib.current_stream()), "eprecon_conv_desc_async")
        return Act(out, relu=relu, acc=acc, eps=eps)
    if aff is None:
        a = torch.empty((2, cout), dtype=torch.float32, device=dev)
        aff = (a[0], a[1])
    assert not isinstance(aff, AccSlice), "an accumulator slice was handed to a launch that cannot produce into it"
    partial = SP.attach_summaries(d, dev)
    nblk, ld = partial.shape[0], d.bn_ld
    _lib.check(lib.eprecon_conv_desc_async(ctypes.byref(d), _lib.current_stream()), "eprecon_conv_desc_async")
    _lib.check(lib.eprecon_batchnorm_finalize_affine_async(
        partial.data_ptr(), nblk, ld, cout, _dptr(gamma), _dptr(beta), float(eps),
        aff[0].data_ptr(), aff[1].data_ptr(), _lib.current_stream()), "eprecon_batchnorm_finalize_affine_async")
    return Act(out, aff[0], aff[1], relu)


def materialize(act, out=None):
    if act.scale is None and act.acc is None:
        if out is not None and out.data_ptr() != act.rows.data_ptr():
            out.copy_(act.rows)
            return out
        return act.rows
    rows = act.rows
    n, c = rows.shape
    if out is None:
        out = torch.empty((n, c), dtype=torch.float32, device=rows.device)
    if act.scale is None and c <= 512:
        _lib.check(_lib.load().eprecon_affine_rows_acc_async(
            rows.data_ptr(), n, c, rows.stride(0), act.acc.block.data_ptr(), act.acc.ld, act.acc.c0, float(act.eps), int(act.relu),
            out.data_ptr(), out.stride(0), _lib.current_stream()), "eprecon_affine_rows_acc_async")
        return out
    act.affine()
    _lib.check(_lib.load().eprecon_affine_rows_async(
        rows.data_ptr(), n, c, rows.stride(0), act.scale.data_ptr(), act.shift.data_ptr(), int(act.relu),
        out.data_ptr(), out.stride(0), _lib.current_stream()), "eprecon_affine_rows_async")
    return out


def _join_rows(name, act, grid, out, out_rows):
    rows = act.rows
    n, c = rows.shape
    assert n == grid.n and act.scale is not None and out.shape == (out_rows, c) and out.stride(1) == 1 and rows.stride(1) == 1
    fn = getattr(_lib.load(), name)
    _lib.check(fn(rows.data_ptr(), grid.maps, grid.height, grid.width, c, rows.stride(0), act.scale.data_ptr(), act.shift.data_ptr(),
                  int(act.relu), out.data_ptr(), out.stride(0), _lib.current_stream()), name)
    return out


def affine_pool2_rows(act, grid, out):
    return _join_rows("eprecon_affine_pool2_rows_async", act, grid, out, grid.maps * (grid.height // 2) * (grid.width // 2))


def affine_up2_rows(act, grid, out):
    return _join_rows("eprecon_affine_up2_rows_async", act, grid, out, grid.maps * 4 * grid.height * grid.width)


def conv_bn(conv, bn, x, grid, out=None, relu=True, pre_relu=False, pre_residual=None):
    res = Act(pre_residual) if pre_residual is not None else None
    return materialize(conv_bn_act(conv, bn, Act(x), grid, relu=relu, pre_relu=pre_relu, residual=res), out=out)
```

### eprecon_amd/modules.py

```python
import math

import torch
import torch.nn as nn
import torch.nn.functional as F

from . import autograd as AG
from . import dense2d as D2
from . import sparse as SP


def recording():
    return torch.is_grad_enabled()

_SETS = SP.IdentityCache(8)


def voxel_set_for(coords, stride=1):
    vs = _SETS.get(coords, int(stride))
    if vs is None:
        c = coords if coords.dtype == torch.int32 else coords.to(torch.int32)
        vs = SP.VoxelSet(c.contiguous(), stride)
        _SETS.put((coords, int(stride), vs))
    return vs


def clear_voxel_set_cache():
    _SETS.clear()


def clear_coordinate_caches():
    clear_voxel_set_cache()
    clear_voxelization_cache()


class SparseSubMConv3d(nn.Module):

    def __init__(self, C_in, C_out, Kernel, Stride=1):
        super().__init__()
        assert Kernel in (1, 3) and Stride == 1
        self.kernel = Kernel
        kvol = Kernel ** 3
        self.weight = nn.Parameter(torch.empty(kvol, C_in, C_out))
        self.bias = nn.Parameter(torch.zeros(C_out))
        self.init_weights()

    def init_weights(self):
        k = self.kernel
        _, cin, cout = self.weight.shape
        bound = math.sqrt(6.0 / (k * k * k * cin + cout * k * k * cin))
        with torch.no_grad():
            self.weight.uniform_(-bound, bound)
            self.bias.zero_()

    @staticmethod
    def from_spconv_layout(w):
        co, k0, k1, k2, ci = w.shape
        return w.permute(3, 2, 1, 4, 0).reshape(k0 * k1 * k2, ci, co)

    def load_spconv_weight(self, w):
        with torch.no_grad():
            self.weight.copy_(self.from_spconv_layout(w))

    def _load_from_state_dict(self, state_dict, prefix, *args, **kwargs):
        for leaf in ("weight", "bias"):
            old = prefix + "sparsesubmconv3d." + leaf
            if old in state_dict:
                state_dict[prefix + leaf] = state_dict.pop(old)
        w = state_dict.get(prefix + "weight")
        if w is not None and w.dim() == 5:
            state_dict[prefix + "weight"] = self.from_spconv_layout(w)
        super()._load_from_state_dict(state_dict, prefix, *args, **kwargs)

    def run(self, features, vset, out=None, relu=False):
        if recording():
            nbr = vset.kernel_map(3) if self.kernel == 3 else None
            y = AG.sparse_conv(features, self.weight, nbr, self.bias)
            y = F.relu(y) if relu else y
            return y if out is None else out.copy_(y)
        nbr = vset.conv_map(3) if self.kernel == 3 else None
        return SP.sparse_conv(features, self.weight, nbr, self.bias, out=out, relu=relu)

    def run_stats(self, features, vset, out=None):
        nbr = vset.conv_map(3) if self.kernel == 3 else None
        return SP.conv_stats(features, self.weight, nbr, out=out, bias=self.bias)

    def run_ln(self, features, vset, ln, out=None, relu=False, residual=None, post_relu=False):
        if recording():
            nbr = vset.kernel_map(3) if self.kernel == 3 else None
            y = AG.sparse_conv(features, self.weight, nbr, self.bias)
            y = F.relu(y) if relu else y
            y = y + residual if residual is not None else y
            y = F.layer_norm(y, ln.normalized_shape, ln.weight, ln.bias, ln.eps)
            y = F.relu(y) if post_relu else y
            return y if out is None else out.copy_(y)
        nbr = vset.conv_map(3) if self.kernel == 3 else None
        return SP.sparse_conv_ln(features, self.weight, nbr, self.bias, ln.weight, ln.bias, ln.eps, out=out,
                                 relu=relu, residual=residual, post_relu=post_relu)

    def forward(self, features, coords, spitial_shape, bs):
        return self.run(features.contiguous(), voxel_set_for(coords))


class _RowLayerNorm(nn.LayerNorm):

    def run(self, x, residual=None, pre_relu=False, post_relu=False, out=None):
        if recording():
            y = F.relu(x) if pre_relu else x
            y = y + residual if residual is not None else y
            y = F.layer_norm(y, self.normalized_shape, self.weight, self.bias, self.eps)
            y = F.relu(y) if post_relu else y
            return y if out is None else out.copy_(y)
        return SP.rowwise_layernorm(x, self.weight, self.bias, self.eps, residual, pre_relu, post_relu, out)


class SubMconv3dBlock(nn.Module):

    def __init__(self, C_in, C_out, Kernel, Stride, Padding):
        super().__init__()
        self.conv = SparseSubMConv3d(C_in, C_out, Kernel, Stride)
        self.ln = _RowLayerNorm(C_out)

    def run(self, x, vset, out=None):
        return self.conv.run_ln(x, vset, self.ln, out=out, post_relu=True)


class Spares3dELAN(nn.Module):

    def __init__(self, dim):
        super().__init__()
        h = dim // 2
        self.conv1 = SubMconv3dBlock(dim, dim, 1, 1, 0)
        self.conv2 = SubMconv3dBlock(dim, dim, 1, 1, 0)
        self.conv3 = SubMconv3dBlock(dim, h, 3, 1, 1)
        self.conv4 = SubMconv3dBlock(h, h, 3, 1, 1)
        self.conv5 = SubMconv3dBlock(h, h, 3, 1, 1)
        self.conv6 = SubMconv3dBlock(h, h, 3, 1, 1)
        self.conv7 = SubMconv3dBlock(dim * 4, dim, 1, 1, 0)
        self.dim = dim

    def run(self, x, vset):
        d, h = self.dim, self.dim // 2
        n = x.shape[0]
        if recording():
            x1, x2 = self.conv1.run(x, vset), self.conv2.run(x, vset)
            x3 = self.conv3.run(x2, vset)
            x4 = self.conv4.run(x3, vset)
            x5 = self.conv5.run(x4, vset)
            x6 = self.conv6.run(x5, vset)
            return self.conv7.run(torch.cat([x1, x2, x3, x4, x5, x6], dim=1), vset)
        cat = torch.empty((n, 4 * d), dtype=torch.float32, device=x.device)
        self.conv1.run(x, vset, out=cat[:, 0:d])
        self.conv2.run(x, vset, out=cat[:, d:2 * d])
        self.conv3.run(cat[:, d:2 * d], vset, out=cat[:, 2 * d:2 * d + h])
        self.conv4.run(cat[:, 2 * d:2 * d + h], vset, out=cat[:, 2 * d + h:3 * d])
        self.conv5.run(cat[:, 2 * d + h:3 * d], vset, out=cat[:, 3 * d:3 * d + h])
        self.conv6.run(cat[:, 3 * d:3 * d + h], vset, out=cat[:, 3 * d + h:4 * d])
        return self.conv7.run(cat, vset)

    def forward(self, voxel_features_o, voxel_coords_bxyz, batch_size, spitial_shape):
        return self.run(voxel_features_o.contiguous(), voxel_set_for(voxel_coords_bxyz))


class SparseConv3d_Residual(nn.Module):

    def __init__(self, dim, Kernel):
        super().__init__()
        self.SConv3d = SparseSubMConv3d(dim, dim, Kernel)
        self.norm = _RowLayerNorm(dim)

    def run(self, x, vset):
        return self.SConv3d.run_ln(x, vset, self.norm, relu=True, residual=x)

    def forward(self, x, coords, spitial_shape, bs):
        return self.run(x.contiguous(), voxel_set_for(coords))


class TrainBatchNorm1d(nn.BatchNorm1d):

    def run(self, x, residual=None, relu=False, out=None):
        if recording():
            y = F.batch_norm(x, self.running_mean, self.running_var, self.weight, self.bias, True, self.momentum, self.eps)
            y = y + residual if residual is not None else y
            y = F.relu(y) if relu else y
            return y if out is None else out.copy_(y)
        return SP.batchnorm_train(x, self.weight, self.bias, self.eps, residual, relu, out)

    def run_partials(self, x, partial, residual=None, relu=False, out=None):
        return SP.batchnorm_apply_partials(x, partial, self.weight, self.bias, self.eps, residual, relu, out)

    def pending_affine(self, partial):
        return SP.bn_affine(partial, self.weight, self.bias, self.eps)


def _rows(x):
    n, c, h, w = x.shape
    return x.permute(0, 2, 3, 1).reshape(n * h * w, c)


def _hip_bn_ok(x):
    return (x.is_cuda and not torch.is_grad_enabled() and x.dim() == 4 and x.shape[1] <= 256
            and x.is_contiguous(memory_format=torch.channels_last) and x.dtype == torch.float32)


def bn2d_train(bn, x, relu=False):
    if _hip_bn_ok(x):
        rows = _rows(x)
        SP.batchnorm_train(rows, bn.weight, bn.bias, bn.eps, relu=relu, out=rows)
        return x
    y = bn(x)
    return F.relu(y) if relu else y


def upsample2x_bilinear(x):
    if x.is_cuda and not torch.is_grad_enabled() and x.shape[1] % 4 == 0 and x.dtype == torch.float32 \
            and x.is_contiguous(memory_format=torch.channels_last):
        from . import _lib
        n, c, h, w = x.shape
        out = torch.empty((n, c, 2 * h, 2 * w), dtype=x.dtype, device=x.device,
                          memory_format=torch.channels_last)
        _lib.check(_lib.load().eprecon_upsample2x_nhwc_async(_lib.ptr(x), _lib.ptr(out), n, h, w, c,
                                                             _lib.current_stream()), "eprecon_upsample2x_nhwc_async")
        return out
    return F.interpolate(x, scale_factor=2, mode="bilinear")
class Conv2d_Block(nn.Module):

    def __init__(self, C_in, C_out, Kernel):
        super().__init__()
        self.conv = nn.Conv2d(C_in, C_out, Kernel, padding="same")
        self.bn = nn.BatchNorm2d(C_out)
        self.act = nn.ReLU()

    def forward(self, x):
        return bn2d_train(self.bn, self.conv(x), relu=True)

    def run_act(self, x, grid, out=None, aff=None):
        return D2.conv_bn_act(self.conv, self.bn, x, grid, out=out, aff=aff, relu=True)

    def run_rows(self, x, grid, out=None):
        return D2.materialize(self.run_act(D2.Act(x), grid), out=out)


class Conv2d_Residual_Block(nn.Module):

    def __init__(self, C, Kernel):
        super().__init__()
        self.conv = nn.Conv2d(C, C, Kernel, padding="same")
        self.bn = nn.BatchNorm2d(C)
        self.relu = nn.ReLU()

    def forward(self, x):
        return bn2d_train(self.bn, x + self.relu(self.conv(x)))

    def run_act(self, x, grid):
        return D2.conv_bn_act(self.conv, self.bn, x, grid, relu=False, pre_relu=True, residual=x)

    def run_rows(self, x, grid, out=None):
        return D2.materialize(self.run_act(D2.Act(x), grid), out=out)


class ELAN(nn.Module):

    def __init__(self, dim):
        super().__init__()
        h = dim // 2
        self.conv1 = Conv2d_Block(dim, dim, 1)
        self.conv2 = Conv2d_Block(dim, dim, 1)
        self.conv3 = Conv2d_Block(dim, h, 3)
        self.conv4 = Conv2d_Block(h, h, 3)
        self.conv5 = Conv2d_Block(h, h, 3)
        self.conv6 = Conv2d_Block(h, h, 3)
        self.conv7 = Conv2d_Block(dim * 4, dim, 1)

    def forward(self, x):
        parts = [self.conv1(x), self.conv2(x)]
        for layer in (self.conv3, self.conv4, self.conv5, self.conv6):
            parts.append(layer(parts[-1]))
        return self.conv7(torch.cat(parts, dim=1))

    def run_act(self, x, grid):
        d = x.rows.shape[1]
        h = d // 2
        dev = x.rows.device
        cat = torch.empty((x.rows.shape[0], 4 * d), dtype=torch.float32, device=dev)
        if D2._ARENA is not None:
            acc = D2.AccSlice.new(4 * d)
            eps = self.conv1.bn.eps
            part = lambda a, b: D2.Act(cat[:, a:b], relu=True, acc=acc.part(a, b), eps=eps)
            sl = lambda a, b: dict(out=cat[:, a:b], aff=acc.part(a, b))
        else:
            aff = torch.empty((2, 4 * d), dtype=torch.float32, device=dev)
            part = lambda a, b: D2.Act(cat[:, a:b], aff[0, a:b], aff[1, a:b], True)
            sl = lambda a, b: dict(out=cat[:, a:b], aff=(aff[0, a:b], aff[1, a:b]))
        self.conv1.run_act(x, grid, **sl(0, d))
        self.conv2.run_act(x, grid, **sl(d, 2 * d))
        self.conv3.run_act(part(d, 2 * d), grid, **sl(2 * d, 2 * d + h))
        self.conv4.run_act(part(2 * d, 2 * d + h), grid, **sl(2 * d + h, 3 * d))
        self.conv5.run_act(part(2 * d + h, 3 * d), grid, **sl(3 * d, 3 * d + h))
        self.conv6.run_act(part(3 * d, 3 * d + h), grid, **sl(3 * d + h, 4 * d))
        return self.conv7.run_act(part(0, 4 * d), grid)

    def run_rows(self, x, grid, out=None):
        return D2.materialize(self.run_act(D2.Act(x), grid), out=out)


class Fusion_Block(nn.Module):

    def __init__(self, C):
        super().__init__()
        self.conv1 = nn.Conv2d(C, C, 3, padding="same")
        self.bn1 = nn.BatchNorm2d(C)
        self.relu = nn.ReLU()
        self.conv2 = nn.Conv2d(C, C, 1, padding="same")
        self.bn2 = nn.BatchNorm2d(C)
        self.ELAN = ELAN(C)

    def forward(self, x):
        x = bn2d_train(self.bn1, self.conv1(x), relu=True)
        x = bn2d_train(self.bn2, self.conv2(x), relu=True)
        return self.ELAN(x)

    def run_act(self, x, grid):
        a = D2.conv_bn_act(self.conv1, self.bn1, D2.Act(x), grid, relu=True)
        a = D2.conv_bn_act(self.conv2, self.bn2, a, grid, relu=True)
        return self.ELAN.run_act(a, grid)

    def run_rows(self, x, grid, out=None):
        return D2.materialize(self.run_act(x, grid), out=out)


def _ln_rows(norm, y, residual=None, pre_relu=False, post_relu=False):
    if y.is_cuda and not torch.is_grad_enabled() and y.dim() == 2 and y.dtype == torch.float32 and y.is_contiguous() \
            and (residual is None or (residual.is_contiguous() and residual.dtype == torch.float32)):
        return SP.rowwise_layernorm(y, norm.weight, norm.bias, norm.eps, residual, pre_relu, post_relu, out=y)
    t = F.relu(y) if pre_relu else y
    if residual is not None:
        t = t + residual
    t = norm(t)
    return F.relu(t) if post_relu else t


_FUSED_HEADS = __import__("os").environ.get("EPRECON_FUSED_HEADS", "1") == "1"


def fused_heads_ok(mod, x):
    return (_FUSED_HEADS and not torch.is_grad_enabled() and x.is_cuda and x.dim() == 2 and x.dtype == torch.float32
            and x.stride(1) == 1 and x.shape[1] == mod.linear1.in_features
            and SP.mlp4x_supported(mod.linear1.in_features, mod.linear3.out_features))


def linear4x_pair(mod_a, mod_b, x):
    if fused_heads_ok(mod_a, x) and mod_a.linear3.out_features == mod_b.linear3.out_features \
            and mod_a.linear1.in_features == mod_b.linear1.in_features:
        ya, yb = SP.mlp4x([mod_a, mod_b], x)
        return ya, yb
    return mod_a(x), mod_b(x)


class Linear4xTrans(nn.Module):

    def __init__(self, C_in, C_out):
        super().__init__()
        self.linear1 = nn.Linear(C_in, C_in * 4)
        self.norm1 = nn.LayerNorm(C_in * 4)
        self.relu = nn.ReLU()
        self.linear2 = nn.Linear(C_in * 4, C_in)
        self.norm2 = nn.LayerNorm(C_in)
        self.linear3 = nn.Linear(C_in, C_out)
        self.use_residual = C_in == C_out
        for lin in (self.linear1, self.linear2, self.linear3):
            nn.init.xavier_uniform_(lin.weight)
            nn.init.zeros_(lin.bias)

    def forward(self, x):
        if recording() and x.is_cuda and x.dim() == 2 and x.dtype == torch.float32:
            lin = lambda layer, t: AG.sparse_conv(t, layer.weight.t(), None, layer.bias)
        else:
            lin = lambda layer, t: layer(t)
# ... 411 lines not shown
```

### eprecon_amd/occupancy_initialization.py

```python
import os

import torch
import torch.nn as nn
import torch.nn.functional as F

from . import _lib
from . import back_project as BP
from .back_project import Back_Project, get_img_feats
from . import dense2d as D2
from . import sparse as SP
from .config import INIT_MIN_VALID
from .modules import (Conv2d_Block, Conv2d_Residual_Block, Fusion_Block, SparseSubMConv3d, Spares3dELAN,
                      TrainBatchNorm1d, _RowLayerNorm, upsample2x_bilinear)


class Occupancy_Initialization(nn.Module):
    def __init__(self, ch_initialization_all, ch_initialization_down, n_views):
        super().__init__()
        ch_all = sum(ch_initialization_all[:3])
        d = ch_initialization_down
        self.self_fusion_1x = Fusion_Block(ch_initialization_all[0])
        self.self_fusion_2x = Fusion_Block(ch_initialization_all[1])
        self.self_fusion_4x = Fusion_Block(ch_initialization_all[2])
        self.ch_down = d
# ... 2 lines not shown
        self.post_fusion_1 = Conv2d_Residual_Block(d, 3)
        self.post_fusion_2 = Conv2d_Residual_Block(d, 3)
        self.post_fusion_3 = Conv2d_Residual_Block(d, 3)
        self.post_fusion_4 = Conv2d_Residual_Block(d, 3)

        self.similary_1 = Spares3dELAN(d)
        self.norm0 = TrainBatchNorm1d(d)
        self.subm1 = SparseSubMConv3d(d, d, 3)
        self.norm1 = _RowLayerNorm(d)
        self.subm2 = SparseSubMConv3d(d, d, 3)
        self.norm2 = _RowLayerNorm(d)
        self.subm3 = SparseSubMConv3d(d, d, 3)
        self.norm3 = _RowLayerNorm(d)
        self.subm4 = SparseSubMConv3d(d, 1, 3)
        self.norm4 = TrainBatchNorm1d(1)
        self.use_hip_graph = os.environ.get("EPRECON_NO_GRAPH", "0") != "1"
        self._graphs = {}
        self.use_hip_conv = os.environ.get("EPRECON_MIOPEN_CONV2D", "0") != "1"
        self._channels_last = False
        self._side_streams = None
        self._bn_arena = None

    def feat_fusion_pre(self, feats_1x, feats_2x, feats_4x):
        if feats_1x.is_cuda and not torch.is_grad_enabled() and self.use_hip_conv:
            return self._feat_fusion_rows(feats_1x, feats_2x, feats_4x)
        if feats_1x.is_cuda and not torch.is_grad_enabled():
            if not self._channels_last:
                for mod in (self.self_fusion_1x, self.self_fusion_2x, self.self_fusion_4x, self.fusion_down,
                            self.post_fusion_1, self.post_fusion_2, self.post_fusion_3, self.post_fusion_4):
                    mod.to(memory_format=torch.channels_last)
                self._channels_last = True
            feats_1x, feats_2x, feats_4x = (t.contiguous(memory_format=torch.channels_last)
                                            for t in (feats_1x, feats_2x, feats_4x))
        f1 = upsample2x_bilinear(self.self_fusion_1x(feats_1x))
        f2 = self.self_fusion_2x(feats_2x)
        f4 = self.pool4x(self.self_fusion_4x(feats_4x))
        x = self.fusion_down(torch.cat([f1, f2, f4], dim=1))
        for blk in (self.post_fusion_1, self.post_fusion_2, self.post_fusion_3, self.post_fusion_4):
            x = blk(x)
        return x

    def _feat_fusion_rows(self, feats_1x, feats_2x, feats_4x):
        return self._fusion_on_rows([D2.rows_of(t.float().contiguous(memory_format=torch.channels_last))
                                     for t in (feats_1x, feats_2x, feats_4x)], [tuple(t.shape) for t in (feats_1x, feats_2x, feats_4x)])

    def _fusion_on_rows(self, rows, shapes):
        dev = rows[0].device
        grids = [D2.PixelGrid.get(v, h, w, dev) for v, c, h, w in shapes]
        g1, g2, g4 = grids
        c1, c2, c4 = (r.shape[1] for r in rows)
        cat = torch.empty((g2.n, c1 + c2 + c4), dtype=torch.float32, device=dev)
        main = torch.cuda.current_stream()
        if self._side_streams is None:
            self._side_streams = (_lib.side_stream(dev, _lib.SIDE_BRANCH_A), _lib.side_stream(dev, _lib.SIDE_BRANCH_B))
        s1, s4 = self._side_streams
        if D2.BN_ACC and self._bn_arena is None:
            self._bn_arena = D2.BnArena(dev)
        with D2.bn_pass(self._bn_arena if D2.BN_ACC else None):
            s1.wait_stream(main)
            s4.wait_stream(main)
            with torch.cuda.stream(s4):
                self._join(self.self_fusion_4x.run_act(rows[2], g4), g4, cat[:, c1 + c2:], pool=True)
            with torch.cuda.stream(s1):
                self._join(self.self_fusion_1x.run_act(rows[0], g1), g1, cat[:, 0:c1], pool=False)
            self.self_fusion_2x.run_rows(rows[1], g2, out=cat[:, c1:c1 + c2])
            main.wait_stream(s1)
            main.wait_stream(s4)
            a = self.fusion_down.run_act(D2.Act(cat), g2)
            for blk in (self.post_fusion_1, self.post_fusion_2, self.post_fusion_3, self.post_fusion_4):
                a = blk.run_act(a, g2)
            return D2.maps_of(D2.materialize(a), g2.maps, g2.height, g2.width)

    def _join(self, act, grid, dst, pool):
        if act.scale is not None and (pool or act.rows.shape[1] % 4 == 0) and _lib.load().eprecon_init_glue():
            return (D2.affine_pool2_rows if pool else D2.affine_up2_rows)(act, grid, dst)
        maps = D2.maps_of(D2.materialize(act), grid.maps, grid.height, grid.width)
        dst[:] = D2.rows_of(self.pool4x(maps) if pool else upsample2x_bilinear(maps))
        return dst

    def _fusion_graphed(self, views):
        key = tuple(tuple(v[0].shape) + (len(v),) for v in views) + (views[0][0].device,)
        direct = self.use_hip_conv and len(views[0]) <= 16 and all(
            m.dtype == torch.float32 and m.is_contiguous() for v in views for m in v)
        key = key + (direct, bool(_lib.load().eprecon_init_glue()))
        entry = self._graphs.get(key)
        if entry is None:
            shapes = [(len(v),) + tuple(v[0].shape) for v in views]
            if direct:
                static_in = [torch.empty((n * h * w, c), dtype=torch.float32, device=views[0][0].device) for n, c, h, w in shapes]
                self._views_to_rows(views, static_in)
                run = lambda: self._fusion_on_rows(static_in, shapes)
            else:
                static_in = [torch.stack(v) for v in views]
                run = lambda: self.feat_fusion_pre(*static_in)
            side = _lib.side_stream(static_in[0].device, _lib.SIDE_SETUP)
            side.wait_stream(torch.cuda.current_stream())
            with torch.cuda.stream(side):
                for _ in range(3):
                    run()
            torch.cuda.current_stream().wait_stream(side)
            graph = torch.cuda.CUDAGraph()
            with torch.cuda.graph(graph, capture_error_mode="thread_local"):
                static_out = run()
            entry = (graph, static_in, static_out)
            self._graphs[key] = entry
        graph, static_in, static_out = entry
        if direct:
            self._views_to_rows(views, static_in)
        else:
            for s_, v in zip(static_in, views):
                torch.stack(v, out=s_)
        graph.replay()
        return static_out

    @staticmethod
    def _views_to_rows(views, rows):
        import ctypes
        d = _lib.ViewsDesc()
        d.levels, d.n_views = len(views), len(views[0])
        for l, (v, r) in enumerate(zip(views, rows)):
            c, h, w = v[0].shape
            d.channels[l], d.hw[l], d.dst[l] = c, h * w, r.data_ptr()
            for i, m in enumerate(v):
                d.src[l][i] = m.data_ptr()
        _lib.check(_lib.load().eprecon_views_to_rows_async(ctypes.byref(d), _lib.current_stream()), "eprecon_views_to_rows_async")

    def sparse_stack(self, var, vset):
        x = self.norm0.run(var)
        x = self.similary_1.run(x, vset)
        for conv, norm in ((self.subm1, self.norm1), (self.subm2, self.norm2), (self.subm3, self.norm3)):
            x = conv.run_ln(x, vset, norm, relu=True, residual=x)
        if torch.is_grad_enabled():
            return self.norm4.run(self.subm4.run(x, vset))
        y, partial = self.subm4.run_stats(x, vset)
        return self.norm4.run_partials(y, partial, out=y)

    def forward(self, coords, origin, voxel_size, features_all, KRcam, shape, stage, min_view_number, between=None):
        bs = features_all[0][0].shape[0]
        dev = features_all[0][0].device
        self.dense_map = None
        on_gpu = dev.type == "cuda" and not torch.is_grad_enabled()
        graphed = self.use_hip_graph and on_gpu
        glue = on_gpu and bool(_lib.load().eprecon_init_glue())
        interval = 2 ** (2 - stage)
        rank = BP.dense_rank_buffer(coords, shape, interval) if glue and bs == 1 else None
        counted = None
        if glue and bs == 1 and self.use_hip_conv:
            h8, w8 = features_all[0][1].shape[-2:]
            counted = BP.count_async(coords, origin, voxel_size, (len(features_all), 1, self.ch_down, h8, w8), KRcam,
                                     min_view_number, BP.MODE_VARIANCE, stream=_lib.side_stream(dev, _lib.SIDE_SETUP))
        per_batch = []
        for b in range(bs):
            views = [[f[l][b] for f in features_all] for l in (2, 1, 0)]
            if graphed:
                fused_b = self._fusion_graphed(views)
                per_batch.append(fused_b if bs == 1 else fused_b.clone())
            else:
                per_batch.append(self.feat_fusion_pre(*[torch.stack(v) for v in views]))
        fused = per_batch[0].unsqueeze(1) if bs == 1 else torch.stack(per_batch, dim=1)
        if on_gpu and (between is not None or glue):
            pend = BP.run_async(coords, origin, voxel_size, fused, KRcam, min_view_number, BP.MODE_VARIANCE,
                                min_valid_per_batch=INIT_MIN_VALID, want_mean=not glue, rank_out=rank, counted=counted)
            if between is not None:
                between()
            res = pend.result()
            if res is not None:
                res["var"] = res.pop("feats")
# ... 20 lines not shown
```

### eprecon_amd/sparse.py

```python
import ctypes
import os
import threading

import torch

from . import _lib


class IdentityCache:

    def __init__(self, max_entries):
        self._max, self._items, self._lock = int(max_entries), [], threading.Lock()

    @staticmethod
    def _key(t, extra):
        return (t.data_ptr(), t._version, t.shape[0], extra)

    def get(self, t, extra=None):
        key = self._key(t, extra)
        with self._lock:
            for k, ref, value in self._items:
                if ref is t and k == key:
                    return value
        return None
# ... 439 lines not shown
        assert dense or (nbr.dtype == torch.int32 and k_map == kvol and nbr.is_contiguous())
    assert c_x == cin and x.dtype == torch.float32
    if out is None:
        out = torch.empty((n_out, cout), dtype=torch.float32, device=x.device)
    assert out.shape == (n_out, cout)
    (ld_x, unit_x), (ld_out, unit_out) = x.stride(), out.stride()
    assert unit_x == 1 and unit_out == 1, "row-major 2-D tensors expected"
    if residual is not None:
        assert residual.shape == (n_out, cout) and residual.dtype == torch.float32
    pack, pack16 = conv_packings(kvol, cout, n_out, nbr is not None, accumulate, 0, k1_min_rows, image_limits)
    if positional and not (dense or (x.is_cuda and ((kvol == 27 and nbr is not None) or pack or pack16))):
        partial = bn_summaries((n_out + 127) // 128, cout, x.device) if stats else None
        _lib.check(lib.eprecon_sparse_conv_fused_async(
            x.data_ptr(), n_in, ld_x, _lib.ptr(nbr), kvol, n_out, _lib.ptr(weight), cin, cout, _lib.ptr(bias),
            _lib.ptr(residual), _ld(residual) if residual is not None else 0, out.data_ptr(), ld_out, int(relu),
            int(accumulate), _lib.ptr(partial), _lib.current_stream()), "eprecon_sparse_conv_fused_async")
        return out, partial, None, None
    d = _lib.ConvDesc()
    d.x, d.n_in, d.ld_x = x.data_ptr(), n_in, ld_x
    d.kvol, d.n_out = kvol, n_out
    d.weight, d.cin, d.cout = weight.data_ptr(), cin, cout
    if bias is not None:
        d.bias = bias.data_ptr()
    if residual is not None:
        d.residual, d.ld_res = residual.data_ptr(), _ld(residual)
        if res_affine is not None:
            d.res_scale, d.res_shift, d.res_relu = _lib.ptr(res_affine[0]), _lib.ptr(res_affine[1]), int(res_affine[2])
    d.out, d.ld_out = out.data_ptr(), ld_out
    if relu:
        d.relu = 1
    if accumulate:
        d.accumulate = 1
    if in_acc is not None:
        acc, eps, in_relu = in_acc
        assert acc.c == cin
        d.in_acc, d.in_acc_ld, d.in_acc_c0, d.in_eps, d.in_relu = acc.block.data_ptr(), acc.ld, acc.c0, float(eps), int(in_relu)
    elif in_affine is not None:
        d.in_scale, d.in_shift, d.in_relu = _lib.ptr(in_affine[0]), _lib.ptr(in_affine[1]), int(in_affine[2])
    if ln is not None:
        assert cout <= 128
        d.ln, d.ln_gamma, d.ln_beta, d.ln_eps, d.ln_post_relu = 1, _lib.ptr(ln[0]), _lib.ptr(ln[1]), float(ln[2]), int(ln[3])
    if image is not None:
        d.img_h, d.img_w, d.img_maps = image
    if dense:
        kind = nbr.describe(d, stats)
        if kind:
            nbr = nbr.rank
            pack, pack16 = conv_packings(kvol, cout, n_out, True, accumulate, kind)
        else:
            nbr = nbr.vset.kernel_map(3)
            d.nbr = nbr.data_ptr()
    elif nbr is not None:
        d.nbr = nbr.data_ptr()
    keep = [weight, nbr]
    if x.is_cuda:
        if pack:
            keep.append(packed_weight(weight))
            d.packed_weight = keep[-1].data_ptr()
        if pack16:
            keep.append(packed_weight16(weight, owner))
            d.packed_weight16 = keep[-1].data_ptr()
    if (kvol == 27 and cin >= 96 and ln is None and d.packed_weight and d.nbr) or (
            d.packed_weight16 and os.environ.get("EPRECON_CONV_PERSIST", "")[:1] == "1"):
        need = int(lib.eprecon_conv_desc_workspace_bytes(ctypes.byref(d)))
        if need:
            keep.append(_lib.workspace(need, x.device))
            d.workspace, d.workspace_bytes = keep[-1].data_ptr(), need
    partial = attach_summaries(d, x.device) if stats else None
    if launch:
        _lib.check(lib.eprecon_conv_desc_async(ctypes.byref(d), _lib.current_stream()), "eprecon_conv_desc_async")
    return out, partial, d, keep


def sparse_conv_fused(x, weight, nbr=None, bias=None, out=None, relu=False, residual=None, accumulate=False,
                      bn_partial=False):
    return conv_call(x, weight, nbr, bias, out, relu, accumulate, residual, stats=bn_partial, positional=True)[:2]


def sparse_conv_ln(x, weight, nbr, bias, ln_weight, ln_bias, ln_eps, out=None, relu=False, residual=None,
                   post_relu=False):
    return conv_call(x, weight, nbr, bias, out, relu, False, residual, ln=(ln_weight, ln_bias, ln_eps, post_relu))[0]


def affine_rows(x, scale, shift, residual=None, relu=False, out=None):
    lib = _lib.load()
    n, c = x.shape
    if out is None:
        out = torch.empty((n, c), dtype=torch.float32, device=x.device)
    _lib.check(lib.eprecon_affine_rows_res_async(
        _lib.ptr(x), n, c, _ld(x), _lib.ptr(scale), _lib.ptr(shift), _lib.ptr(residual),
        _ld(residual) if residual is not None else 0, int(relu), _lib.ptr(out), _ld(out), _lib.current_stream()),
        "eprecon_affine_rows_res_async")
    return out


def conv_stats(x, weight, nbr=None, in_affine=None, out=None, bias=None):
    rows = x.shape[0] if nbr is None else nbr.shape[1]
    return conv_call(x, weight, nbr, bias, out, in_affine=in_affine, stats=True, launch=rows > 0)[:2]


def bn_affine(partial, gamma, beta, eps):
    lib = _lib.load()
    c = partial.shape[2]
    nblk, ld = summary_layout(partial)
    aff = torch.empty((2, c), dtype=torch.float32, device=partial.device)
    _lib.check(lib.eprecon_batchnorm_finalize_affine_async(
        partial.data_ptr(), nblk, ld, c, _lib.ptr(gamma), _lib.ptr(beta), float(eps), aff[0].data_ptr(),
        aff[1].data_ptr(), _lib.current_stream()), "eprecon_batchnorm_finalize_affine_async")
    return aff[0], aff[1]


def batchnorm_apply_partials(x, partial, gamma=None, beta=None, eps=1e-5, residual=None, relu=False, out=None,
                             res_affine=None):
    lib = _lib.load()
    n, c = x.shape
    assert partial.shape[1:] == (3, c)
    nblk, ld = summary_layout(partial)
    if out is None:
        out = torch.empty((n, c), dtype=torch.float32, device=x.device)
    ws = torch.empty((lib.eprecon_batchnorm_apply_workspace_bytes(c),), dtype=torch.uint8, device=x.device)
    if res_affine is not None:
        _lib.check(lib.eprecon_batchnorm_apply_partials_res_async(
            _lib.ptr(x), n, c, _ld(x), _lib.ptr(partial), nblk, ld, _lib.ptr(gamma), _lib.ptr(beta), float(eps),
            _lib.ptr(residual), _ld(residual), _lib.ptr(res_affine[0]), _lib.ptr(res_affine[1]), int(relu), _lib.ptr(out),
            _ld(out), _lib.ptr(ws), ws.numel(), _lib.current_stream()), "eprecon_batchnorm_apply_partials_res_async")
        return out
    _lib.check(lib.eprecon_batchnorm_apply_partials_async(
        _lib.ptr(x), n, c, _ld(x), _lib.ptr(partial), nblk, ld, _lib.ptr(gamma), _lib.ptr(beta),
        float(eps), _lib.ptr(residual), _ld(residual) if residual is not None else 0, int(relu), _lib.ptr(out),
        _ld(out), None, None, _lib.ptr(ws), ws.numel(), _lib.current_stream()),
        "eprecon_batchnorm_apply_partials_async")
    return out


def batchnorm_train(x, gamma=None, beta=None, eps=1e-5, residual=None, relu=False, out=None):
    lib = _lib.load()
    n, c = x.shape
    if out is None:
        out = torch.empty((n, c), dtype=torch.float32, device=x.device)
    ws = _lib.workspace(lib.eprecon_batchnorm_workspace_bytes(n, c), x.device)
    _lib.check(lib.eprecon_batchnorm_train_async(
        _lib.ptr(x), n, c, _ld(x), _lib.ptr(gamma), _lib.ptr(beta), float(eps), _lib.ptr(residual),
        _ld(residual) if residual is not None else 0, int(relu), _lib.ptr(out), _ld(out), None, None,
        _lib.ptr(ws), ws.numel(), _lib.current_stream()), "eprecon_batchnorm_train_async")
    return out


def rowwise_layernorm(x, gamma=None, beta=None, eps=1e-5, residual=None, pre_relu=False, post_relu=False,
                      out=None):
    lib = _lib.load()
    n, c = x.shape
    if out is None:
        out = torch.empty((n, c), dtype=torch.float32, device=x.device)
    _lib.check(lib.eprecon_rowwise_layernorm_async(
        _lib.ptr(x), n, c, _ld(x), _lib.ptr(residual), _ld(residual) if residual is not None else 0,
        _lib.ptr(gamma), _lib.ptr(beta), float(eps), int(pre_relu), int(post_relu), _lib.ptr(out),
        _ld(out), _lib.current_stream()), "eprecon_rowwise_layernorm_async")
    return out


def _pack_mlp_weight(wt):
    k, m = wt.shape
    kc, mt = (k + 15) // 16, (m + 15) // 16
    w = torch.zeros((16 * kc, 16 * mt), dtype=torch.float32, device=wt.device)
    w[:k, :m] = wt
    return w.view(kc, 4, 4, mt, 16).permute(3, 0, 1, 4, 2).contiguous().view(-1)
# ... 58 lines not shown
```

### include/eprecon_hip.h

```cpp
#ifndef EPRECON_HIP_H
#define EPRECON_HIP_H

#include <stddef.h>
#include <stdint.h>

#ifdef __cplusplus
extern "C" {
#endif

#define EPRECON_OK 0
#define EPRECON_EMPTY 1
#define EPRECON_ERR_ARG (-1)
#define EPRECON_ERR_WORKSPACE (-2)
#define EPRECON_ERR_UNSUPPORTED (-3)
#define EPRECON_ERR_HIP_BASE (-1000)

#define EPRECON_ABI_VERSION 1
int eprecon_abi_version(void);
const char *eprecon_build_arch(void);

#define EPRECON_BP_MEAN 0
#define EPRECON_BP_MEAN_DEPTH 1
#define EPRECON_BP_VARIANCE 2

// ... 56 lines not shown
const char *eprecon_profile_last_conv_kernel(void);
int eprecon_profile_mark_async(int id, void *stream);

int eprecon_nchw_to_nhwc_async(const float *in, float *out, int maps, int channels, int hw,
                               void *stream);
typedef struct eprecon_views_desc {
    const float *src[3][16];
    float *dst[3];
    int32_t channels[3]; int32_t hw[3];
    int32_t levels; int32_t n_views;
} eprecon_views_desc;
int eprecon_views_to_rows_async(const eprecon_views_desc *desc, void *stream);

uint32_t eprecon_hash_capacity(int64_t n);
size_t eprecon_hash_table_bytes(uint32_t capacity);
int eprecon_hash_build_async(const int32_t *coords, int64_t n, int quantum, void *table,
                             uint32_t capacity, void *stream);
int eprecon_hash_build_dn_async(const int32_t *coords, int64_t n_cap, const int32_t *n_dev, int quantum, void *table,
                                uint32_t capacity, void *stream);
int eprecon_hash_query_async(const void *table, uint32_t capacity, const int32_t *queries, int64_t m,
                             int quantum, int32_t *out_index, void *stream);
int eprecon_hash_status(const void *table, void *stream);

size_t eprecon_unique_workspace_bytes(int64_t n);
size_t eprecon_exclusive_scan_scratch_ints(int64_t n);
int eprecon_exclusive_scan_async(const int32_t *in, int64_t n, int32_t *out, int32_t *total, int32_t *scratch, void *stream);
int eprecon_unique_coords_async(const int32_t *coords, int64_t n, int quantum, void *table,
                                uint32_t capacity, int32_t *inverse, int32_t *unique_coords,
                                int32_t *n_unique_dev, void *workspace, size_t workspace_bytes,
                                void *stream);

int eprecon_unique_coords_dn_async(const int32_t *coords, int64_t n_cap, const int32_t *n_dev, int quantum, void *table,
                                   uint32_t capacity, int32_t *inverse, int32_t *unique_coords, int32_t *n_unique_dev,
                                   void *workspace, size_t workspace_bytes, void *stream);
int eprecon_unique_hierarchy_dn_async(const int32_t *coords, int64_t n_cap, const int32_t *n_dev, int levels, void *const *tables,
                                      const uint32_t *capacities, int32_t *const *inverse, int32_t *const *unique_coords,
                                      int32_t *summary, void *workspace, size_t workspace_bytes, void *stream);

int eprecon_kernel_map_self_async(const void *table, uint32_t capacity, const int32_t *coords, int64_t n, int stride, int32_t *nbr,
                                  void *stream);

size_t eprecon_components_workspace_bytes(int64_t n);
int eprecon_components_async(const int32_t *nbr, int64_t n, const int32_t *keys, int connectivity, int32_t *label, int32_t *status,
                             void *workspace, size_t workspace_bytes, void *stream);
int eprecon_kernel_map_async(const void *table, uint32_t capacity, const int32_t *coords, int64_t n,
                             int ksize, int stride, int32_t *nbr, void *stream);
int eprecon_transpose_map_async(const int32_t *fine_coords, int64_t n, const int32_t *parent,
                                int fine_stride, int32_t *up_map, void *stream);
int eprecon_sparse_conv_async(const float *x, int64_t n_in, int ld_x, const int32_t *nbr, int kvol,
                              int64_t n_out, const float *weight, int cin, int cout, const float *bias,
                              float *out, int ld_out, int relu, int accumulate, void *stream);
size_t eprecon_conv_bn_partial_bytes(int64_t n_out, int cout);
int eprecon_sparse_conv_fused_async(const float *x, int64_t n_in, int ld_x, const int32_t *nbr, int kvol,
                                    int64_t n_out, const float *weight, int cin, int cout,
                                    const float *bias, const float *residual, int ld_res, float *out,
                                    int ld_out, int relu, int accumulate, float *bn_partial, void *stream);
typedef struct eprecon_conv_desc {
    const float *x; int64_t n_in; int ld_x;
    const int32_t *nbr; int kvol; int64_t n_out;
    const float *weight; int cin; int cout;
    const float *bias;
    const float *residual; int ld_res;
    float *out; int ld_out;
    int relu; int accumulate;
    const float *in_scale; const float *in_shift; int in_relu;
    const float *res_scale; const float *res_shift; int res_relu;
    float *bn_partial; int bn_ld;
    int ln; const float *ln_gamma; const float *ln_beta; float ln_eps; int ln_post_relu;
    int img_h; int img_w; int img_maps;
    const int32_t *vox_rank; int grid_x; int grid_y; int grid_z;
    const float *packed_weight;
    const float *packed_weight16;
    void *workspace; size_t workspace_bytes;
    long long *bn_acc; int bn_acc_ld; int bn_acc_c0; const float *bn_gamma; const float *bn_beta;
    const long long *in_acc; int in_acc_ld; int in_acc_c0; float in_eps; float *in_affine_scratch;
} eprecon_conv_desc;
size_t eprecon_bn_acc_words(int ld);
int eprecon_conv_desc_takes_bn_acc(const eprecon_conv_desc *desc);
int eprecon_batchnorm_acc_affine_async(const long long *acc, int acc_ld, int acc_c0, int channels, float eps, float *scale_out,
                                       float *shift_out, void *stream);
int eprecon_affine_rows_acc_async(const float *x, int64_t n, int channels, int ld_x, const long long *acc, int acc_ld, int acc_c0,
                                  float eps, int relu, float *out, int ld_out, void *stream);
int eprecon_conv_desc_async(const eprecon_conv_desc *desc, void *stream);
size_t eprecon_conv_desc_workspace_bytes(const eprecon_conv_desc *desc);
int64_t eprecon_conv_desc_partial_rows(const eprecon_conv_desc *desc);
int eprecon_conv_dense3d_kind(const eprecon_conv_desc *desc);
int eprecon_batchnorm_finalize_affine_async(const float *partial, int64_t nblk, int64_t ld, int channels, const float *gamma,
                                            const float *beta, float eps, float *scale_out, float *shift_out,
                                            void *stream);
int eprecon_affine_rows_async(const float *x, int64_t n, int channels, int ld_x, const float *scale,
                              const float *shift, int relu, float *out, int ld_out, void *stream);
int eprecon_affine_pool2_rows_async(const float *x, int maps, int height, int width, int channels, int ld_x, const float *scale,
                                    const float *shift, int relu, float *out, int ld_out, void *stream);
int eprecon_affine_up2_rows_async(const float *x, int maps, int height, int width, int channels, int ld_x, const float *scale,
                                  const float *shift, int relu, float *out, int ld_out, void *stream);
int eprecon_affine_rows_res_async(const float *x, int64_t n, int channels, int ld_x, const float *scale,
                                  const float *shift, const float *residual, int ld_res, int relu, float *out,
                                  int ld_out, void *stream);
int eprecon_pixel_map_async(int maps, int height, int width, int ksize, int32_t *nbr, void *stream);
int eprecon_grid_rank_async(const int32_t *coords, int64_t n, int stride, int grid_x, int grid_y, int grid_z, int32_t *rank,
                            void *stream);
size_t eprecon_conv_pack_weight_floats(int kvol, int cin, int cout);
int eprecon_conv_pack_weight_async(const float *weight, int kvol, int cin, int cout, float *packed, void *stream);
size_t eprecon_conv_pack_weight16_floats(int kvol, int cin, int cout);
int eprecon_conv_pack_weight16_async(const float *weight, int kvol, int cin, int cout, float *packed, void *stream);
typedef struct eprecon_pack_job {
    const float *weight; float *packed;
    int32_t kvol; int32_t cin; int32_t cout; int32_t kind;
} eprecon_pack_job;
int eprecon_conv_pack_many_async(const eprecon_pack_job *jobs, int njobs, void *stream);

size_t eprecon_batchnorm_workspace_bytes(int64_t n, int channels);
int eprecon_batchnorm_train_async(const float *x, int64_t n, int channels, int ld_x, const float *gamma,
                                  const float *beta, float eps, const float *residual, int ld_res,
                                  int relu, float *out, int ld_out, float *mean_out, float *var_out,
                                  void *workspace, size_t workspace_bytes, void *stream);
size_t eprecon_batchnorm_apply_workspace_bytes(int channels);
int eprecon_batchnorm_apply_partials_async(const float *x, int64_t n, int channels, int ld_x,
                                           const float *partial, int64_t nblk, int64_t ld, const float *gamma,
                                           const float *beta, float eps, const float *residual,
                                           int ld_res, int relu, float *out, int ld_out, float *mean_out,
                                           float *var_out, void *workspace, size_t workspace_bytes,
                                           void *stream);
int eprecon_batchnorm_apply_partials_res_async(const float *x, int64_t n, int channels, int ld_x, const float *partial,
                                               int64_t nblk, int64_t ld, const float *gamma, const float *beta, float eps,
                                               const float *residual, int ld_res, const float *res_scale,
                                               const float *res_shift, int relu, float *out, int ld_out, void *workspace,
                                               size_t workspace_bytes, void *stream);
int eprecon_rowwise_layernorm_async(const float *x, int64_t n, int channels, int ld_x,
                                    const float *residual, int ld_res, const float *gamma,
                                    const float *beta, float eps, int pre_relu, int post_relu,
                                    float *out, int ld_out, void *stream);

size_t eprecon_init_select_workspace_bytes(int batch, int dim);
int eprecon_init_select_async(const float *logit, const int32_t *coords, int64_t n, float threshold,
                              int batch, int dim, int cell, int32_t *out_coords, int32_t *n_out_dev,
                              void *workspace, size_t workspace_bytes, void *stream);
int eprecon_init_select_dense_async(const float *logit, const int32_t *coords, int64_t n, const int32_t *rank, int grid_x,
                                    int grid_y, int grid_z, int stride, float threshold, int dim, int cell,
                                    int32_t *out_coords, int32_t *n_out_dev, void *workspace, size_t workspace_bytes,
                                    void *stream);
size_t eprecon_sparsify_workspace_bytes(int64_t n);
int eprecon_sparsify_async(const float *occ, int ld_occ, float threshold, const unsigned char *target,
                           const int32_t *coords, const float *tsdf, int ld_tsdf, const float *feat_all, int ld_feat,
                           int c_all, int c_feat, int64_t n, int batch, int32_t *out_coords, float *out_tsdf,
                           float *out_occ, float *out_all, float *out_feat, int32_t *counts, void *workspace,
                           size_t workspace_bytes, void *stream);
int eprecon_upsample_async(const float *feat, int ld_feat, const int32_t *coords, int64_t n, int channels,
                           int interval, float *up_feat, int32_t *up_coords, void *stream);

int eprecon_aligned_coords_async(const int32_t *coords, int64_t n, const float *origin, int batch,
                                 float voxel_size, const float *world_to_aligned_camera, float *out_xyzb,
                                 void *stream);
int eprecon_point_quantize_async(const float *points_xyzb, int64_t n, float resolution, float *scaled_xyzb,
                                 int32_t *voxel_bxyz, void *stream);
int eprecon_spvcnn_points_dn_async(const int32_t *src_coords, int64_t cap_src, const int32_t *n_src_dev, int children,
                                   int interval, const float *origin, int batch, float voxel_size,
                                   const float *world_to_aligned_camera, float resolution, int32_t *up_coords, float *r_coords,
                                   float *scaled_xyzb, int32_t *voxel_bxyz, int32_t *n_points_dev, void *stream);
int eprecon_point_quantize_dn_async(const float *points_xyzb, int64_t n_cap, const int32_t *n_dev, float resolution,
                                    float *scaled_xyzb, int32_t *voxel_bxyz, void *stream);
size_t eprecon_segment_workspace_bytes(int64_t n, int64_t m);
int eprecon_segment_lists_async(const int32_t *idx, int64_t n, int64_t m, int32_t *offsets, int32_t *order,
                                void *workspace, size_t workspace_bytes, void *stream);
int eprecon_segment_mean_async(const float *feat, int ld_feat, const int32_t *offsets, const int32_t *order,
                               int64_t m, int channels, float *out, int ld_out, void *stream);
int eprecon_sphash_async(const int32_t *coords, int64_t n, int64_t *out_hash, void *stream);
size_t eprecon_sphash_order_workspace_bytes(int64_t n);
int eprecon_sphash_order_async(const int32_t *coords, int64_t n, int32_t *perm_out, int32_t *rank_out, void *workspace,
                               size_t workspace_bytes, void *stream);
int eprecon_remap_index_async(const int32_t *idx, int64_t n, const int32_t *rank_old, const int32_t *perm_new,
                              int64_t m_new, int32_t *out, void *stream);
// ... 365 lines not shown
```

Baseline: 819.1.

## Batch sibling ELAN convolutions sharing input into one paired launch

Adds a paired convolution path in which two convolutions that share the same input, neighbor map and shape run in a single kernel launch. blockIdx.y selects the second layer's weights, outputs and norm parameters, and the two BN finalize launches are merged the same way. The ELAN blocks' conv1/conv2 calls (both the 3D and 2D variants) go through this path. The goal is fewer launches and better GPU fill for small grids, capped by a workgroup limit. The cost is extra dispatch complexity plus a fallback to sequential launches when the two layers don't match.

```diff
diff --git a/eprecon_amd/_lib.py b/eprecon_amd/_lib.py
--- a/eprecon_amd/_lib.py
+++ b/eprecon_amd/_lib.py
@@ -49,6 +49,10 @@
     "eprecon_sparse_conv_fused_async": (_i, [_vp, _i64, _i, _vp, _i, _i64, _vp, _i, _i, _vp, _vp, _i, _vp, _i, _i, _i,
                                              _vp, _vp]),
     "eprecon_conv_desc_async": (_i, [_vp, _vp]),
+    "eprecon_conv_desc_pair_async": (_i, [_vp, _vp, _vp]),
+    "eprecon_conv_desc_pairable": (_i, [_vp, _vp]),
+    "eprecon_conv_pair_enabled": (_i, []),
+    "eprecon_batchnorm_finalize_affine_pair_async": (_i, [_vp, _vp, _i64, _i64, _i, _vp, _vp, _vp, _vp, _f, _vp, _vp, _vp, _vp, _vp]),
     "eprecon_exclusive_scan_scratch_ints": (_sz, [_i64]),
     "eprecon_exclusive_scan_async": (_i, [_vp, _i64, _vp, _vp, _vp, _vp]),
     "eprecon_conv_desc_partial_rows": (_i64, [_vp]),
diff --git a/eprecon_amd/csrc/conv_common.hpp b/eprecon_amd/csrc/conv_common.hpp
--- a/eprecon_amd/csrc/conv_common.hpp
+++ b/eprecon_amd/csrc/conv_common.hpp
@@ -43,6 +43,20 @@
     float in_eps;
 };
 
+struct ConvPair {
+    const float *w, *wq, *wq16, *bias;
+    float *out, *bn_partial;
+    const float *ln_gamma, *ln_beta;
+};
+
+__device__ __forceinline__ void conv_pair_select(ConvParams &p, const ConvPair &b, unsigned job)
+{
+    if (job == 0) return;
+    p.w = b.w; p.wq = b.wq; p.wq16 = b.wq16; p.bias = b.bias;
+    p.out = b.out; p.bn_partial = b.bn_partial;
+    p.ln_gamma = b.ln_gamma; p.ln_beta = b.ln_beta;
+}
+
 constexpr int kBnCopies = 8, kBnWords = 7;
 #ifndef EP_BN_ABL
 #define EP_BN_ABL 0
@@ -281,11 +295,13 @@
 int launch_resident_narrow(const ConvParams &p, hipStream_t st);
 bool resident_wide_ok(const ConvParams &p);
 int launch_resident_wide(const ConvParams &p, hipStream_t st);
-int launch_mfma(const ConvParams &p, hipStream_t st);
+int launch_mfma(const ConvParams &p, hipStream_t st, const ConvPair *pair = nullptr);
+bool mfma_pair_ok(const ConvParams &p);
 
 bool direct16_ok(const ConvParams &p);
 constexpr int kDirectRows = 128;
-int launch_direct16(const ConvParams &p, hipStream_t st);
+int launch_direct16(const ConvParams &p, hipStream_t st, const ConvPair *pair = nullptr);
+bool direct16_pair_ok(const ConvParams &p);
 int direct16_partial_block_rows(const ConvParams &p);
 size_t direct16_workspace_bytes(const ConvParams &p);
 
diff --git a/eprecon_amd/csrc/norm.hip b/eprecon_amd/csrc/norm.hip
--- a/eprecon_amd/csrc/norm.hip
+++ b/eprecon_amd/csrc/norm.hip
@@ -118,11 +118,20 @@
     }
 }
 
+struct BnFinalizeSecond {
+    const float *partial, *gamma, *beta;
+    float *scale_out, *shift_out;
+};
+
 template <int NU>
 __global__ __launch_bounds__(256) void bn_finalize_affine_kernel(const float *partial, int nblk, int64_t ld, int C,
                                                                  const float *gamma, const float *beta, float eps,
-                                                                 float *scale_out, float *shift_out)
-{
+                                                                 float *scale_out, float *shift_out, BnFinalizeSecond second)
+{
+    if (blockIdx.y) {
+        partial = second.partial; gamma = second.gamma; beta = second.beta;
+        scale_out = second.scale_out; shift_out = second.shift_out;
+    }
     __shared__ float sN[4], sMean[4], sM2[4];
     const int c = blockIdx.x, tid = threadIdx.x;
     const float g_c = gamma ? gamma[c] : 1.0f, b_c = beta ? beta[c] : 0.0f;
@@ -506,23 +515,43 @@
                              mean, var, (hipStream_t)stream, res_scale, res_shift);
 }
 
+static int bn_finalize_affine_launch(const float *partial, int64_t nblk, int64_t ld, int channels, const float *gamma,
+                                     const float *beta, float eps, float *scale_out, float *shift_out,
+                                     const BnFinalizeSecond *second, hipStream_t st)
+{
+    const dim3 grid(channels, second ? 2 : 1);
+    const BnFinalizeSecond b = second ? *second : BnFinalizeSecond{};
+    switch (bn_finalize_nu(nblk)) {
+#define EP_FINALIZE(NU)                                                                                                          \
+    case NU:                                                                                                                     \
+        hipLaunchKernelGGL(bn_finalize_affine_kernel<NU>, grid, dim3(256), 0, st, partial, (int)nblk, ld, channels, gamma, beta, \
+                           eps, scale_out, shift_out, b);                                                                        \
+        break
+        EP_FINALIZE(1); EP_FINALIZE(2); EP_FINALIZE(4); EP_FINALIZE(8); EP_FINALIZE(16);
+#undef EP_FINALIZE
+    }
+    EP_LAUNCH_CHECK();
+    return EPRECON_OK;
+}
+
 int eprecon_batchnorm_finalize_affine_async(const float *partial, int64_t nblk, int64_t ld, int channels, const float *gamma,
                                             const float *beta, float eps, float *scale_out, float *shift_out,
                                             void *stream)
 {
     if (!partial || !scale_out || !shift_out || nblk <= 0 || nblk > 0x7fffffff || ld < nblk || channels <= 0) return EPRECON_ERR_ARG;
-    hipStream_t st = (hipStream_t)stream;
-    switch (bn_finalize_nu(nblk)) {
-#define EP_FINALIZE(NU)                                                                                                            \
-    case NU:                                                                                                                       \
-        hipLaunchKernelGGL(bn_finalize_affine_kernel<NU>, dim3(channels), dim3(256), 0, st, partial, (int)nblk, ld, channels, gamma, \
-                           beta, eps, scale_out, shift_out);                                                                         \
-        break
-        EP_FINALIZE(1); EP_FINALIZE(2); EP_FINALIZE(4); EP_FINALIZE(8); EP_FINALIZE(16);
-#undef EP_FINALIZE
-    }
-    EP_LAUNCH_CHECK();
-    return EPRECON_OK;
+    return bn_finalize_affine_launch(partial, nblk, ld, channels, gamma, beta, eps, scale_out, shift_out, nullptr, (hipStream_t)stream);
+}
+
+int eprecon_batchnorm_finalize_affine_pair_async(const float *partial_a, const float *partial_b, int64_t nblk, int64_t ld,
+                                                 int channels, const float *gamma_a, const float *beta_a, const float *gamma_b,
+                                                 const float *beta_b, float eps, float *scale_a, float *shift_a, float *scale_b,
+                                                 float *shift_b, void *stream)
+{
+    if (!partial_a || !partial_b || !scale_a || !shift_a || !scale_b || !shift_b || nblk <= 0 || nblk > 0x7fffffff || ld < nblk ||
+        channels <= 0)
+        return EPRECON_ERR_ARG;
+    const BnFinalizeSecond second = {partial_b, gamma_b, beta_b, scale_b, shift_b};
+    return bn_finalize_affine_launch(partial_a, nblk, ld, channels, gamma_a, beta_a, eps, scale_a, shift_a, &second, (hipStream_t)stream);
 }
 
 int eprecon_affine_rows_async(const float *x, int64_t n, int channels, int ld_x, const float *scale,
diff --git a/eprecon_amd/csrc/sparse_conv.hip b/eprecon_amd/csrc/sparse_conv.hip
--- a/eprecon_amd/csrc/sparse_conv.hip
+++ b/eprecon_amd/csrc/sparse_conv.hip
@@ -228,8 +228,9 @@
     return n_in > 0 ? ((n_in - 1) * (int64_t)p.ld_x + ((p.Cin + 3) & ~3)) * 4 : 0;
 }
 
-static int conv_check_and_run(ConvParams &p, int64_t n_in, int64_t n_out, void *stream)
-{
+static int conv_check(ConvParams &p, int64_t n_in, int64_t n_out, bool *run)
+{
+    *run = false;
     if (!p.x || !p.w || !p.out || n_in < 0 || n_out < 0 || p.K <= 0 || p.K > 64 || p.Cin <= 0 || p.Cout <= 0 ||
         p.ld_x < p.Cin || p.ld_out < p.Cout || (p.res && p.ld_res < p.Cout))
         return EPRECON_ERR_ARG;
@@ -241,7 +242,15 @@
     if (n_out == 0) return EPRECON_OK;
     p.n_out = (int)n_out;
     p.x_bytes = conv_x_bytes(p, n_in);
-    return conv_dispatch(p, (hipStream_t)stream);
+    *run = true;
+    return EPRECON_OK;
+}
+
+static int conv_check_and_run(ConvParams &p, int64_t n_in, int64_t n_out, void *stream)
+{
+    bool run = false;
+    const int rc = conv_check(p, n_in, n_out, &run);
+    return rc == EPRECON_OK && run ? conv_dispatch(p, (hipStream_t)stream) : rc;
 }
 
 static void params_from_desc(ConvParams &p, const eprecon_conv_desc *d)
@@ -341,6 +350,70 @@
     return query_params(p, d) ? select_conv(p).partial_rows : 0;
 }
 
+constexpr int64_t kPairMaxWorkgroups = 2700;
+
+static int64_t pair_max_workgroups()
+{
+    const char *e = getenv("EPRECON_CONV_PAIR_MAX_WG");
+    return e && *e ? atoll(e) : kPairMaxWorkgroups;
+}
+
+extern "C" int eprecon_conv_pair_enabled(void) { return ep::switch_off("EPRECON_CONV_PAIR") ? 0 : 1; }
+
+static bool pair_resolve(ConvParams &pa, ConvParams &pb, const eprecon_conv_desc *a, const eprecon_conv_desc *b, ConvFamily *family)
+{
+    if (!eprecon_conv_pair_enabled() || !query_params(pa, a) || !query_params(pb, b)) return false;
+    if (g_conv_prof.armed || getenv("EPRECON_CONV_LOG")) return false;
+    if (a->n_in != b->n_in || a->n_out != b->n_out) return false;
+    if (pa.bn_acc || pb.bn_acc || pa.in_acc || pb.in_acc) return false;
+    const bool same =
+        pa.x == pb.x && pa.ld_x == pb.ld_x && pa.nbr == pb.nbr && pa.K == pb.K && pa.Cin == pb.Cin && pa.Cout == pb.Cout &&
+        pa.ld_out == pb.ld_out && pa.relu == pb.relu && pa.accumulate == pb.accumulate && pa.res == pb.res && pa.ld_res == pb.ld_res &&
+        pa.res_scale == pb.res_scale && pa.res_shift == pb.res_shift && pa.res_relu == pb.res_relu && pa.in_scale == pb.in_scale &&
+        pa.in_shift == pb.in_shift && pa.in_relu == pb.in_relu && pa.ln == pb.ln && pa.ln_eps == pb.ln_eps &&
+        pa.ln_post_relu == pb.ln_post_relu && pa.img_h == pb.img_h && pa.img_w == pb.img_w && pa.img_maps == pb.img_maps &&
+        pa.vox_rank == pb.vox_rank && pa.gx == pb.gx && pa.gy == pb.gy && pa.gz == pb.gz && pa.bn_ld == pb.bn_ld &&
+        (pa.bn_partial == nullptr) == (pb.bn_partial == nullptr) && (pa.wq == nullptr) == (pb.wq == nullptr) &&
+        (pa.wq16 == nullptr) == (pb.wq16 == nullptr);
+    if (!same || pa.out == pb.out || (pa.bn_partial && pa.bn_partial == pb.bn_partial)) return false;
+    const ConvChoice ca = select_conv(pa), cb = select_conv(pb);
+    if (ca.status != EPRECON_OK || cb.status != EPRECON_OK || ca.family != cb.family || ca.partial_rows != cb.partial_rows) return false;
+    if (pa.bn_partial) {
+        if (pa.bn_ld == 0) pa.bn_ld = pb.bn_ld = (int)(ca.partial_rows > 0 ? ca.partial_rows : 1);
+        if (pa.bn_ld < ca.partial_rows) return false;
+    }
+    int64_t workgroups = 0;
+    if (ca.family == kFamDirect16 && direct16_pair_ok(pa) && direct16_pair_ok(pb))
+        workgroups = 2 * ceil_div((int64_t)pa.n_out, (int64_t)kDirectRows);
+    else if (ca.family == kFamMfma && mfma_pair_ok(pa) && mfma_pair_ok(pb))
+        workgroups = 2 * ceil_div((int64_t)pa.n_out, (int64_t)kRowsPerBlock) * ceil_div((int64_t)pa.Cout, (int64_t)32);
+    if (workgroups == 0 || workgroups > pair_max_workgroups()) return false;
+    bool run_a = false, run_b = false;
+    if (conv_check(pa, a->n_in, a->n_out, &run_a) != EPRECON_OK || conv_check(pb, b->n_in, b->n_out, &run_b) != EPRECON_OK) return false;
+    *family = ca.family;
+    return run_a && run_b;
+}
+
+extern "C" int eprecon_conv_desc_pairable(const eprecon_conv_desc *a, const eprecon_conv_desc *b)
+{
+    ConvParams pa = {}, pb = {};
+    ConvFamily family = kFamMfma;
+    return pair_resolve(pa, pb, a, b, &family) ? 1 : 0;
+}
+
+extern "C" int eprecon_conv_desc_pair_async(const eprecon_conv_desc *a, const eprecon_conv_desc *b, void *stream)
+{
+    ConvParams pa = {}, pb = {};
+    ConvFamily family = kFamMfma;
+    if (!pair_resolve(pa, pb, a, b, &family)) {
+        const int rc = eprecon_conv_desc_async(a, stream);
+        return rc != EPRECON_OK ? rc : eprecon_conv_desc_async(b, stream);
+    }
+    const ConvPair second = {pb.w, pb.wq, pb.wq16, pb.bias, pb.out, pb.bn_partial, pb.ln_gamma, pb.ln_beta};
+    g_last_conv_kernel = kConvFamilyNames[family];
+    return family == kFamDirect16 ? launch_direct16(pa, (hipStream_t)stream, &second) : launch_mfma(pa, (hipStream_t)stream, &second);
+}
+
 extern "C" int eprecon_sparse_conv_fused_async(const float *x, int64_t n_in, int ld_x, const int32_t *nbr,
                                                int kvol, int64_t n_out, const float *weight, int cin,
                                                int cout, const float *bias, const float *residual,
diff --git a/eprecon_amd/csrc/sparse_conv_direct.hip b/eprecon_amd/csrc/sparse_conv_direct.hip
--- a/eprecon_amd/csrc/sparse_conv_direct.hip
+++ b/eprecon_amd/csrc/sparse_conv_direct.hip
@@ -1,10 +1,10 @@
 #include "sparse_conv_direct_select.hpp"
 
 namespace epconv {
-int launch_direct16_ct1(const ConvParams &p, hipStream_t st);
-int launch_direct16_ct2(const ConvParams &p, hipStream_t st);
-int launch_direct16_ct3(const ConvParams &p, hipStream_t st);
-int launch_direct16_ct4(const ConvParams &p, hipStream_t st);
+int launch_direct16_ct1(const ConvParams &p, hipStream_t st, const ConvPair *pair);
+int launch_direct16_ct2(const ConvParams &p, hipStream_t st, const ConvPair *pair);
+int launch_direct16_ct3(const ConvParams &p, hipStream_t st, const ConvPair *pair);
+int launch_direct16_ct4(const ConvParams &p, hipStream_t st, const ConvPair *pair);
 
 bool direct16_ok(const ConvParams &p)
 {
@@ -22,13 +22,15 @@
 int direct16_partial_block_rows(const ConvParams &p) { return persist_shape_ok(p) ? kJobRows : kDirectRows; }
 size_t direct16_workspace_bytes(const ConvParams &p) { return persist_shape_ok(p) ? kPersistCtrBytes : 0; }
 
-int launch_direct16(const ConvParams &p, hipStream_t st)
+bool direct16_pair_ok(const ConvParams &p) { return (p.Cin + 15) / 16 <= 6 && !persist_shape_ok(p); }
+
+int launch_direct16(const ConvParams &p, hipStream_t st, const ConvPair *pair)
 {
     switch ((p.Cout + 15) / 16) {
-        case 1: return launch_direct16_ct1(p, st);
-        case 2: return launch_direct16_ct2(p, st);
-        case 3: return launch_direct16_ct3(p, st);
-        default: return launch_direct16_ct4(p, st);
+        case 1: return launch_direct16_ct1(p, st, pair);
+        case 2: return launch_direct16_ct2(p, st, pair);
+        case 3: return launch_direct16_ct3(p, st, pair);
+        default: return launch_direct16_ct4(p, st, pair);
     }
 }
 
diff --git a/eprecon_amd/csrc/sparse_conv_direct_ct1.hip b/eprecon_amd/csrc/sparse_conv_direct_ct1.hip
--- a/eprecon_amd/csrc/sparse_conv_direct_ct1.hip
+++ b/eprecon_amd/csrc/sparse_conv_direct_ct1.hip
@@ -1,5 +1,5 @@
 #include "sparse_conv_direct_launch.hpp"
 
 namespace epconv {
-int launch_direct16_ct1(const ConvParams &p, hipStream_t st) { return launch_ct<1>(p, st); }
+int launch_direct16_ct1(const ConvParams &p, hipStream_t st, const ConvPair *pair) { return launch_ct<1>(p, st, pair); }
 }
diff --git a/eprecon_amd/csrc/sparse_conv_direct_ct2.hip b/eprecon_amd/csrc/sparse_conv_direct_ct2.hip
--- a/eprecon_amd/csrc/sparse_conv_direct_ct2.hip
+++ b/eprecon_amd/csrc/sparse_conv_direct_ct2.hip
@@ -1,5 +1,5 @@
 #include "sparse_conv_direct_launch.hpp"
 
 namespace epconv {
-int launch_direct16_ct2(const ConvParams &p, hipStream_t st) { return launch_ct<2>(p, st); }
+int launch_direct16_ct2(const ConvParams &p, hipStream_t st, const ConvPair *pair) { return launch_ct<2>(p, st, pair); }
 }
diff --git a/eprecon_amd/csrc/sparse_conv_direct_ct3.hip b/eprecon_amd/csrc/sparse_conv_direct_ct3.hip
--- a/eprecon_amd/csrc/sparse_conv_direct_ct3.hip
+++ b/eprecon_amd/csrc/sparse_conv_direct_ct3.hip
@@ -1,5 +1,5 @@
 #include "sparse_conv_direct_launch.hpp"
 
 namespace epconv {
-int launch_direct16_ct3(const ConvParams &p, hipStream_t st) { return launch_ct<3>(p, st); }
+int launch_direct16_ct3(const ConvParams &p, hipStream_t st, const ConvPair *pair) { return launch_ct<3>(p, st, pair); }
 }
diff --git a/eprecon_amd/csrc/sparse_conv_direct_ct4.hip b/eprecon_amd/csrc/sparse_conv_direct_ct4.hip
--- a/eprecon_amd/csrc/sparse_conv_direct_ct4.hip
+++ b/eprecon_amd/csrc/sparse_conv_direct_ct4.hip
@@ -1,5 +1,5 @@
 #include "sparse_conv_direct_launch.hpp"
 
 namespace epconv {
-int launch_direct16_ct4(const ConvParams &p, hipStream_t st) { return launch_ct<4>(p, st); }
+int launch_direct16_ct4(const ConvParams &p, hipStream_t st, const ConvPair *pair) { return launch_ct<4>(p, st, pair); }
 }
diff --git a/eprecon_amd/csrc/sparse_conv_direct_kernels.hpp b/eprecon_amd/csrc/sparse_conv_direct_kernels.hpp
--- a/eprecon_amd/csrc/sparse_conv_direct_kernels.hpp
+++ b/eprecon_amd/csrc/sparse_conv_direct_kernels.hpp
@@ -5,9 +5,10 @@
 namespace {
 
 template <int CT, int KCH, bool TAIL = false, int G = stage_chunks(KCH), bool BF = false, int MODE = 0>
-__global__ __launch_bounds__(256) void spconv_direct16_kernel(ConvParams p)
+__global__ __launch_bounds__(256) void spconv_direct16_kernel(ConvParams p, ConvPair second)
 {
     extern __shared__ __attribute__((aligned(16))) char smem[];
+    conv_pair_select(p, second, blockIdx.y);
     constexpr int RT = kRT, ROWS = kDirectRows;
     constexpr int CTM = TAIL ? CT - 1 : CT;
     constexpr int CTA = CTM > 0 ? CTM : 1;
diff --git a/eprecon_amd/csrc/sparse_conv_direct_launch.hpp b/eprecon_amd/csrc/sparse_conv_direct_launch.hpp
--- a/eprecon_amd/csrc/sparse_conv_direct_launch.hpp
+++ b/eprecon_amd/csrc/sparse_conv_direct_launch.hpp
@@ -6,17 +6,18 @@
 namespace {
 
 template <int CT, int KCH>
-int launch_form(const DirectForm &f, const ConvParams &p, dim3 grid, size_t lds, hipStream_t st)
+int launch_form(const DirectForm &f, const ConvParams &p, dim3 grid, size_t lds, hipStream_t st, const ConvPair *pair)
 {
     constexpr int G0 = stage_chunks(KCH), GA = alt_stage_chunks(KCH);
     if (f.persist) {
+        if (pair) return EPRECON_ERR_UNSUPPORTED;
         if constexpr (KCH * (CT * 1024 - 512) <= 4864) {
             if (f.tail) return launch_persist<CT, KCH, true>(p, st);
             if constexpr (KCH * CT * 1024 <= 4864) return launch_persist<CT, KCH, false>(p, st);
         }
         return EPRECON_ERR_UNSUPPORTED;
     }
-    void (*kern)(ConvParams) = nullptr;
+    void (*kern)(ConvParams, ConvPair) = nullptr;
     auto with_tail = [&](auto tail) {
         constexpr bool TAIL = decltype(tail)::value;
         if (f.bf) {
@@ -38,7 +39,8 @@
     if (f.tail) with_tail(std::true_type{});
     else with_tail(std::false_type{});
     if (!kern) return EPRECON_ERR_UNSUPPORTED;
-    hipLaunchKernelGGL(kern, grid, dim3(256), lds, st, p);
+    if (pair) grid.y = 2;
+    hipLaunchKernelGGL(kern, grid, dim3(256), lds, st, p, pair ? *pair : ConvPair{});
     EP_LAUNCH_CHECK();
     return EPRECON_OK;
 }
@@ -65,21 +67,22 @@
 }
 
 template <int CT, int KCH>
-int launch_k(const ConvParams &p, hipStream_t st)
+int launch_k(const ConvParams &p, hipStream_t st, const ConvPair *pair)
 {
     const size_t lds = direct_lds_bytes(p.K, CT, KCH);
     const DirectSwitches sw = direct_switches();
     int occ_p = 1, occ_a = 1;
     if constexpr (alt_stage_chunks(KCH) != 0) stage_occupancy<CT, KCH>(direct_tail(p, sw), lds, occ_p, occ_a);
     const DirectForm f = select_direct_form(p, sw, device_cus(), occ_p, occ_a);
-    return launch_form<CT, KCH>(f, p, dim3((unsigned)ceil_div(p.n_out, kDirectRows)), lds, st);
+    return launch_form<CT, KCH>(f, p, dim3((unsigned)ceil_div(p.n_out, kDirectRows)), lds, st, pair);
 }
 
 template <int CT>
-int launch_ct(const ConvParams &p, hipStream_t st)
+int launch_ct(const ConvParams &p, hipStream_t st, const ConvPair *pair)
 {
     const int kch = (p.Cin + 15) / 16;
-    if (kch <= 6) return pick<1, 2, 3, 4, 5, 6>(kch, [&](auto k) { return launch_k<CT, decltype(k)::value>(p, st); });
+    if (kch <= 6) return pick<1, 2, 3, 4, 5, 6>(kch, [&](auto k) { return launch_k<CT, decltype(k)::value>(p, st, pair); });
+    if (pair) return EPRECON_ERR_UNSUPPORTED;
     hipLaunchKernelGGL((spconv_direct16_generic_kernel<CT>), dim3((unsigned)ceil_div(p.n_out, kDirectRows)), dim3(256),
                        direct_lds_bytes(p.K, CT, kch), st, p, kch);
     EP_LAUNCH_CHECK();
diff --git a/eprecon_amd/csrc/sparse_conv_slab.hip b/eprecon_amd/csrc/sparse_conv_slab.hip
--- a/eprecon_amd/csrc/sparse_conv_slab.hip
+++ b/eprecon_amd/csrc/sparse_conv_slab.hip
@@ -7,9 +7,10 @@
 using namespace epconv;
 
 template <int NT, bool VEC4>
-__global__ __launch_bounds__(256) void spconv_mfma_kernel(ConvParams p)
+__global__ __launch_bounds__(256) void spconv_mfma_kernel(ConvParams p, ConvPair second)
 {
     extern __shared__ __attribute__((aligned(16))) char smem[];
+    conv_pair_select(p, second, blockIdx.z);
     constexpr int TN = 32 * NT;
     float *sW = reinterpret_cast<float *>(smem);
     int *sNbr = reinterpret_cast<int *>(sW + 2 * kSlabC * TN);
@@ -107,16 +108,17 @@
 }
 
 template <int NT>
-int launch_conv(const ConvParams &p, bool vec4, hipStream_t st)
-{
-    const dim3 grid((unsigned)ceil_div(p.n_out, kRowsPerBlock), (unsigned)ceil_div(p.Cout, 32 * NT));
+int launch_conv(const ConvParams &p, bool vec4, hipStream_t st, const ConvPair *pair = nullptr)
+{
+    const dim3 grid((unsigned)ceil_div(p.n_out, kRowsPerBlock), (unsigned)ceil_div(p.Cout, 32 * NT), pair ? 2 : 1);
+    const ConvPair second = pair ? *pair : ConvPair{};
     const size_t lds = (size_t)2 * kSlabC * 32 * NT * sizeof(float) +
                        (size_t)p.K * kRowsPerBlock * sizeof(int) + (size_t)((p.K + 3) & ~3) * sizeof(int) +
                        (size_t)2 * ((p.Cin + 3) & ~3) * sizeof(float) + 16;
     if (vec4)
-        hipLaunchKernelGGL((spconv_mfma_kernel<NT, true>), grid, dim3(256), lds, st, p);
+        hipLaunchKernelGGL((spconv_mfma_kernel<NT, true>), grid, dim3(256), lds, st, p, second);
     else
-        hipLaunchKernelGGL((spconv_mfma_kernel<NT, false>), grid, dim3(256), lds, st, p);
+        hipLaunchKernelGGL((spconv_mfma_kernel<NT, false>), grid, dim3(256), lds, st, p, second);
     EP_LAUNCH_CHECK();
     return EPRECON_OK;
 }
@@ -298,11 +300,14 @@
     return two ? launch_resident_nt2(p, gather_vec4(p), cin_pad8(p), st) : launch_resident_nt1(p, gather_vec4(p), cin_pad8(p), st);
 }
 
-int launch_mfma(const ConvParams &p, hipStream_t st)
+bool mfma_pair_ok(const ConvParams &p) { return gather_vec4(p) && ((p.Cout + 31) / 32 == 1 || column_split(p)); }
+
+int launch_mfma(const ConvParams &p, hipStream_t st, const ConvPair *pair)
 {
     const bool vec4 = gather_vec4(p);
     const int nt_full = (p.Cout + 31) / 32;
-    if (nt_full == 1 || column_split(p)) return launch_conv<1>(p, vec4, st);
+    if (pair && !mfma_pair_ok(p)) return EPRECON_ERR_UNSUPPORTED;
+    if (nt_full == 1 || column_split(p)) return launch_conv<1>(p, vec4, st, pair);
     if (nt_full == 2) return launch_conv<2>(p, vec4, st);
     if (nt_full == 3) return launch_conv<3>(p, vec4, st);
     return launch_conv<4>(p, vec4, st);
diff --git a/eprecon_amd/dense2d.py b/eprecon_amd/dense2d.py
--- a/eprecon_amd/dense2d.py
+++ b/eprecon_amd/dense2d.py
@@ -150,19 +150,23 @@
                           out=out, aff=aff, relu=relu, pre_relu=pre_relu, residual=residual)
 
 
-def conv_bn_launch(w, bias, gamma, beta, eps, k, x, grid, out=None, aff=None, relu=True, pre_relu=False,
-                   residual=None):
-    lib = _lib.load()
-    cout = w.shape[2]
-    dev = x.rows.device
+def _conv_bn_desc(w, bias, k, x, grid, out, pre_relu, residual):
     acc_in = x.acc is not None and x.scale is None
-    out, _, d, _keep = SP.conv_call(
+    return SP.conv_call(
         x.rows, w, grid.kernel_map(k), bias, out, relu=pre_relu, residual=None if residual is None else residual.rows,
         res_affine=None if residual is None else (*residual.affine(), residual.relu),
         in_affine=(x.scale, x.shift, x.relu) if x.scale is not None or x.relu else None,
         in_acc=(x.acc, x.eps, x.relu) if acc_in else None,
         image=(grid.height, grid.width, grid.maps) if k == 3 else None, launch=False, k1_min_rows=K1_DIRECT_2D_MIN_ROWS,
         image_limits=(DIRECT_2D_MIN_ROWS, SHORT_2D_MAX_ROWS, SHORT_2D_MAX_COUT) if k == 3 else None)
+
+
+def conv_bn_launch(w, bias, gamma, beta, eps, k, x, grid, out=None, aff=None, relu=True, pre_relu=False,
+                   residual=None):
+    lib = _lib.load()
+    cout = w.shape[2]
+    dev = x.rows.device
+    out, _, d, _keep = _conv_bn_desc(w, bias, k, x, grid, out, pre_relu, residual)
     if _ARENA is not None and (aff is None or isinstance(aff, AccSlice)) and lib.eprecon_conv_desc_takes_bn_acc(ctypes.byref(d)):
         acc = aff if aff is not None else AccSlice.new(cout)
         assert acc.c == cout
@@ -181,6 +185,33 @@
         partial.data_ptr(), nblk, ld, cout, _dptr(gamma), _dptr(beta), float(eps),
         aff[0].data_ptr(), aff[1].data_ptr(), _lib.current_stream()), "eprecon_batchnorm_finalize_affine_async")
     return Act(out, aff[0], aff[1], relu)
+
+
+def conv_bn_act_pair(layer_a, layer_b, x, grid, outs, affs, relu=True):
+    lib = _lib.load()
+    (conv_a, bn_a), (conv_b, bn_b) = layer_a, layer_b
+    if (_ARENA is not None or x.acc is not None or bn_a.eps != bn_b.eps or conv_a.kernel_size != conv_b.kernel_size
+            or not lib.eprecon_conv_pair_enabled()):
+        return tuple(conv_bn_act(c, b, x, grid, out=o, aff=a, relu=relu) for (c, b), o, a in zip((layer_a, layer_b), outs, affs))
+    dev, st = x.rows.device, _lib.current_stream()
+    k = conv_a.kernel_size[0]
+    calls = [_conv_bn_desc(packed_weight(c), c.bias, k, x, grid, o, False, None) for (c, _), o in zip((layer_a, layer_b), outs)]
+    (da, db), cout = (calls[0][2], calls[1][2]), calls[0][2].cout
+    parts = [SP.attach_summaries(d, dev) for d in (da, db)]
+    nblk, ld = parts[0].shape[0], da.bn_ld
+    if lib.eprecon_conv_desc_pairable(ctypes.byref(da), ctypes.byref(db)):
+        _lib.check(lib.eprecon_conv_desc_pair_async(ctypes.byref(da), ctypes.byref(db), st), "eprecon_conv_desc_pair_async")
+        _lib.check(lib.eprecon_batchnorm_finalize_affine_pair_async(
+            parts[0].data_ptr(), parts[1].data_ptr(), nblk, ld, cout, _dptr(bn_a.weight), _dptr(bn_a.bias), _dptr(bn_b.weight),
+            _dptr(bn_b.bias), float(bn_a.eps), affs[0][0].data_ptr(), affs[0][1].data_ptr(), affs[1][0].data_ptr(),
+            affs[1][1].data_ptr(), st), "eprecon_batchnorm_finalize_affine_pair_async")
+    else:
+        for d, part, (_, bn), aff in zip((da, db), parts, (layer_a, layer_b), affs):
+            _lib.check(lib.eprecon_conv_desc_async(ctypes.byref(d), st), "eprecon_conv_desc_async")
+            _lib.check(lib.eprecon_batchnorm_finalize_affine_async(
+                part.data_ptr(), part.shape[0], d.bn_ld, cout, _dptr(bn.weight), _dptr(bn.bias), float(bn.eps),
+                aff[0].data_ptr(), aff[1].data_ptr(), st), "eprecon_batchnorm_finalize_affine_async")
+    return tuple(Act(c[0], aff[0], aff[1], relu) for c, aff in zip(calls, affs))
 
 
 def materialize(act, out=None):
diff --git a/eprecon_amd/modules.py b/eprecon_amd/modules.py
--- a/eprecon_amd/modules.py
+++ b/eprecon_amd/modules.py
@@ -97,6 +97,12 @@
         return SP.sparse_conv_ln(features, self.weight, nbr, self.bias, ln.weight, ln.bias, ln.eps, out=out,
                                  relu=relu, residual=residual, post_relu=post_relu)
 
+    def run_ln_pair(self, other, features, vset, ln, other_ln, outs, post_relu=False):
+        assert not recording() and self.kernel == other.kernel and self.weight.shape == other.weight.shape
+        nbr = vset.conv_map(3) if self.kernel == 3 else None
+        return SP.sparse_conv_ln_pair(features, nbr, [(c.weight, c.bias, n.weight, n.bias, n.eps) for c, n in ((self, ln), (other, other_ln))],
+                                      outs, post_relu=post_relu)
+
     def forward(self, features, coords, spitial_shape, bs):
         return self.run(features.contiguous(), voxel_set_for(coords))
 
@@ -122,6 +128,9 @@
 
     def run(self, x, vset, out=None):
         return self.conv.run_ln(x, vset, self.ln, out=out, post_relu=True)
+
+    def run_pair(self, other, x, vset, outs):
+        return self.conv.run_ln_pair(other.conv, x, vset, self.ln, other.ln, outs, post_relu=True)
 
 
 class Spares3dELAN(nn.Module):
@@ -149,8 +158,7 @@
             x6 = self.conv6.run(x5, vset)
             return self.conv7.run(torch.cat([x1, x2, x3, x4, x5, x6], dim=1), vset)
         cat = torch.empty((n, 4 * d), dtype=torch.float32, device=x.device)
-        self.conv1.run(x, vset, out=cat[:, 0:d])
-        self.conv2.run(x, vset, out=cat[:, d:2 * d])
+        self.conv1.run_pair(self.conv2, x, vset, (cat[:, 0:d], cat[:, d:2 * d]))
         self.conv3.run(cat[:, d:2 * d], vset, out=cat[:, 2 * d:2 * d + h])
         self.conv4.run(cat[:, 2 * d:2 * d + h], vset, out=cat[:, 2 * d + h:3 * d])
         self.conv5.run(cat[:, 2 * d + h:3 * d], vset, out=cat[:, 3 * d:3 * d + h])
@@ -291,8 +299,12 @@
             aff = torch.empty((2, 4 * d), dtype=torch.float32, device=dev)
             part = lambda a, b: D2.Act(cat[:, a:b], aff[0, a:b], aff[1, a:b], True)
             sl = lambda a, b: dict(out=cat[:, a:b], aff=(aff[0, a:b], aff[1, a:b]))
-        self.conv1.run_act(x, grid, **sl(0, d))
-        self.conv2.run_act(x, grid, **sl(d, 2 * d))
+        if D2._ARENA is None:
+            D2.conv_bn_act_pair((self.conv1.conv, self.conv1.bn), (self.conv2.conv, self.conv2.bn), x, grid,
+                                (cat[:, 0:d], cat[:, d:2 * d]), ((aff[0, 0:d], aff[1, 0:d]), (aff[0, d:2 * d], aff[1, d:2 * d])))
+        else:
+            self.conv1.run_act(x, grid, **sl(0, d))
+            self.conv2.run_act(x, grid, **sl(d, 2 * d))
         self.conv3.run_act(part(d, 2 * d), grid, **sl(2 * d, 2 * d + h))
         self.conv4.run_act(part(2 * d, 2 * d + h), grid, **sl(2 * d + h, 3 * d))
         self.conv5.run_act(part(2 * d + h, 3 * d), grid, **sl(3 * d, 3 * d + h))
diff --git a/eprecon_amd/occupancy_initialization.py b/eprecon_amd/occupancy_initialization.py
--- a/eprecon_amd/occupancy_initialization.py
+++ b/eprecon_amd/occupancy_initialization.py
@@ -108,7 +108,7 @@
         key = tuple(tuple(v[0].shape) + (len(v),) for v in views) + (views[0][0].device,)
         direct = self.use_hip_conv and len(views[0]) <= 16 and all(
             m.dtype == torch.float32 and m.is_contiguous() for v in views for m in v)
-        key = key + (direct, bool(_lib.load().eprecon_init_glue()))
+        key = key + (direct, bool(_lib.load().eprecon_init_glue()), bool(_lib.load().eprecon_conv_pair_enabled()))
         entry = self._graphs.get(key)
         if entry is None:
             shapes = [(len(v),) + tuple(v[0].shape) for v in views]
diff --git a/eprecon_amd/sparse.py b/eprecon_amd/sparse.py
--- a/eprecon_amd/sparse.py
+++ b/eprecon_amd/sparse.py
@@ -545,6 +545,14 @@
     return conv_call(x, weight, nbr, bias, out, relu, False, residual, ln=(ln_weight, ln_bias, ln_eps, post_relu))[0]
 
 
+def sparse_conv_ln_pair(x, nbr, layers, outs, relu=False, post_relu=False):
+    calls = [conv_call(x, w, nbr, b, out, relu, False, None, ln=(lw, lb, eps, post_relu), launch=False)
+             for (w, b, lw, lb, eps), out in zip(layers, outs)]
+    _lib.check(_lib.load().eprecon_conv_desc_pair_async(ctypes.byref(calls[0][2]), ctypes.byref(calls[1][2]), _lib.current_stream()),
+               "eprecon_conv_desc_pair_async")
+    return calls[0][0], calls[1][0]
+
+
 def affine_rows(x, scale, shift, residual=None, relu=False, out=None):
     lib = _lib.load()
     n, c = x.shape
diff --git a/include/eprecon_hip.h b/include/eprecon_hip.h
--- a/include/eprecon_hip.h
+++ b/include/eprecon_hip.h
@@ -162,12 +162,19 @@
 int eprecon_affine_rows_acc_async(const float *x, int64_t n, int channels, int ld_x, const long long *acc, int acc_ld, int acc_c0,
                                   float eps, int relu, float *out, int ld_out, void *stream);
 int eprecon_conv_desc_async(const eprecon_conv_desc *desc, void *stream);
+int eprecon_conv_desc_pair_async(const eprecon_conv_desc *a, const eprecon_conv_desc *b, void *stream);
+int eprecon_conv_desc_pairable(const eprecon_conv_desc *a, const eprecon_conv_desc *b);
+int eprecon_conv_pair_enabled(void);
 size_t eprecon_conv_desc_workspace_bytes(const eprecon_conv_desc *desc);
 int64_t eprecon_conv_desc_partial_rows(const eprecon_conv_desc *desc);
 int eprecon_conv_dense3d_kind(const eprecon_conv_desc *desc);
 int eprecon_batchnorm_finalize_affine_async(const float *partial, int64_t nblk, int64_t ld, int channels, const float *gamma,
                                             const float *beta, float eps, float *scale_out, float *shift_out,
                                             void *stream);
+int eprecon_batchnorm_finalize_affine_pair_async(const float *partial_a, const float *partial_b, int64_t nblk, int64_t ld,
+                                                 int channels, const float *gamma_a, const float *beta_a, const float *gamma_b,
+                                                 const float *beta_b, float eps, float *scale_a, float *shift_a, float *scale_b,
+                                                 float *shift_b, void *stream);
 int eprecon_affine_rows_async(const float *x, int64_t n, int channels, int ld_x, const float *scale,
                               const float *shift, int relu, float *out, int ld_out, void *stream);
 int eprecon_affine_pool2_rows_async(const float *x, int maps, int height, int width, int channels, int ld_x, const float *scale,
```

New measurement: 830.7 (median of 6 runs). +1.4%, better.
